# ChampiB/CBO_with_OOP

Measured on AMD Instinct MI355X. Metric: candidate-intervention acquisitions/sec (16k grid, d=3), higher is better.
Workload: dtype f64

## Files before the change

cbo_with_oop_amd/csrc/cbo_api.hip:

```cpp
#include <algorithm>
#include <atomic>
#include <cmath>
#include <cstdio>
#include <cstdlib>
#include <chrono>
#include <cstring>
#include <mutex>
#include <string>
#include <map>
#include <utility>
#include <vector>

#include "cbo_internal.h"
#include "schedule_tuner.h"

using namespace cbo;

static thread_local std::string g_err;
static std::atomic<uint64_t> g_fit_stamp{0};

static int fail(int code, const std::string &msg)
{
    g_err = msg;
    return code;
}
namespace cbo {
int set_error(int code, const std::string &msg) { return fail(code, msg); }
}

static std::mutex g_live_mutex;
static std::vector<cbo_ctx *> g_live;
static void shutdown_all_at_exit()
{
    for (;;) {
        cbo_ctx *c = nullptr;
        {
            std::lock_guard<std::mutex> lock(g_live_mutex);
            if (g_live.empty()) break;
            c = g_live.back();
        }
        cbo_shutdown(c);
    }
}

#define HIP_TRY(expr)                                                                                   \
    do {                                                                                                \
        hipError_t e_ = (expr);                                                                         \
        if (e_ != hipSuccess)                                                                           \
            return fail(CBO_ERR_HIP, std::string(#expr) + ": " + hipGetErrorString(e_));                \
    } while (0)

constexpr size_t kStageBytes = 64 << 10;

enum Phase { PH_KXX = 0, PH_CHOL, PH_ALPHA, PH_KSTAR, PH_TRSM, PH_ACQ, PH_CONVERT, PH_COUNT };

struct EventPair {
    hipEvent_t a, b;
    int phase;
};

template <class T, bool Pinned = false>
struct GrowBuf {
    T *p = nullptr;
    size_t cap = 0;
    GrowBuf() = default;
    GrowBuf(const GrowBuf &) = delete;
    GrowBuf &operator=(const GrowBuf &) = delete;
    ~GrowBuf() { release(); }
    operator T *() const { return p; }
    void release() { if (p) Pinned ? hipHostFree(p) : hipFree(p); p = nullptr; cap = 0; }
};
template <class T>
using PinnedBuf = GrowBuf<T, true>;

struct cbo_ctx {
    int device = 0;
    hipStream_t stream = nullptr;
    hipStream_t side_stream = nullptr;
    hipStream_t sweep_stream = nullptr;
    hipStream_t bulk_stream = nullptr;
    std::vector<hipEvent_t> chol_events;
    std::vector<hipEvent_t> pipe_events;
    hipEvent_t ev_join = nullptr, ev_join2 = nullptr, ev_fork = nullptr;
    hipEvent_t region_a = nullptr, region_b = nullptr;
    double pipe_tail_frac = -1.0;
    int pipe_group = 0;
    int pipe_lead = -1;
    CholOptions chol;
    int vec_solve_form = 2;
    int n_cu = 256;
    int n_cu_pipe = 256;
    ScheduleTable schedule;
    int64_t fused_fallbacks = 0;
    bool sweep_cache = true;
    bool small_sets = true;
    int sweep_mode = -1;
    int overlap_mode = -1;
    bool profiling = false;
    std::vector<EventPair> pending;
    EventPair pipe_cur{};
    std::vector<hipEvent_t> pool;
    cbo_timers timers{};
    GrowBuf<double> V;
    GrowBuf<double> W;
    GrowBuf<double> gpart;
    GrowBuf<double> mupart;
    PinnedBuf<cbo_small_set> sets_host;
    PinnedBuf<cbo_small_result> small_out;
    GrowBuf<double> small_scratch;
    GrowBuf<double> small_part_val; GrowBuf<int64_t> small_part_idx;
    GrowBuf<int> small_info;
    int small_seq = 0;
    int polled_launches = 0;
    PinnedBuf<cbo_small_lml_result> lml_out;
    PinnedBuf<cbo_small_lml_result> lml_batch_out;
    PinnedBuf<cbo_small_loo_result> loo_out;
    int loo_route = 0;
    PinnedBuf<double> hyper_host;
    PinnedBuf<HyperSet> hyper_sets_host;
    GrowBuf<double> hyper_sum;
    PinnedBuf<cbo_small_aux> aux_host;
    PinnedBuf<double> mes_host;
    GrowBuf<double> gumbel_mean, gumbel_var, gumbel_out;
    GrowBuf<int64_t> gumbel_status;
    PinnedBuf<GumbelSet> gumbel_sets_host;
    int hyper_schedule = 0;
    GrowBuf<double> q, mu, mean, var, acq;
    double *part_val = nullptr; int64_t *part_idx = nullptr;
    double *best_val = nullptr; int64_t *best_idx = nullptr;
    double *h_best_val = nullptr; int64_t *h_best_idx = nullptr;
    int *h_info = nullptr;
    cbo_cands *scratch_k = nullptr;
    GrowBuf<double> grads;
    GrowBuf<double> export_buf;
    GrowBuf<double> cov;
    GrowBuf<double> samp_A, samp_invDt;
    GrowBuf<int> samp_info;
    GrowBuf<double> samp_Z, samp_out;
    GrowBuf<double> ivr_part;
    GrowBuf<double> con_terms;
    GrowBuf<double> plugin_y;
    GrowBuf<double> batch_W, batch_q, batch_col, batch_part;
    GrowBuf<double> append_part;
    GrowBuf<BatchState> batch_state;
    PinnedBuf<double> batch_h_vals; PinnedBuf<int64_t> batch_h_idxs;
    double *stage = nullptr; hipEvent_t stage_done = nullptr; bool stage_pending = false;
    size_t max_ws_bytes = (size_t)32 << 30;
    char name[128] = {0};
};

struct cbo_gp {
    cbo_ctx *ctx = nullptr;
    int64_t n = 0, n_pad = 0, lda = 0;
    int d = 0;
    PointSet X;
    double *raw = nullptr;
    double *y = nullptr, *ls_dev = nullptr;
    std::vector<double> ls;
    std::vector<double> h_pv;
    KernelHyper h{};
    double noise_var = 0.0;
    double *A = nullptr;
    double *invDt = nullptr;
    double *alpha = nullptr;
    double *z = nullptr;
    int *info = nullptr;
    bool fitted = false;
    uint64_t fit_stamp = 0;
    bool alpha_ready = false;
    int tries = 0;
    double jitter = 0.0;
    uint64_t parent_stamp = 0;
    double append_d = 0.0, append_zn = 0.0;
    double *lvec = nullptr;
    cbo_cands *probe = nullptr;
    int k_last = 1;
// ... 103 lines not shown
        float ms = 0.f;
        hipEventElapsedTime(&ms, p.a, p.b);
        switch (p.phase) {
            case PH_KXX: c->timers.ms_kxx += ms; break;
            case PH_CHOL: c->timers.ms_chol += ms; break;
            case PH_ALPHA: c->timers.ms_alpha += ms; break;
            case PH_KSTAR: c->timers.ms_kstar += ms; break;
            case PH_TRSM: c->timers.ms_trsm += ms; break;
            case PH_ACQ: c->timers.ms_acq += ms; break;
            case PH_CONVERT: c->timers.ms_f32_convert += ms; break;
        }
        c->pool.push_back(p.a);
        c->pool.push_back(p.b);
    }
    c->pending.clear();
}

static void destroy_ctx(cbo_ctx *c);

extern "C" int cbo_abi_version(void) { return CBO_HIP_ABI_VERSION; }
extern "C" const char *cbo_last_error(void) { return g_err.c_str(); }

extern "C" int cbo_device_count(int *count_out)
{
    if (!count_out) return fail(CBO_ERR_INVALID, "count_out is NULL");
    int n = 0;
    hipError_t e = hipGetDeviceCount(&n);
    if (e != hipSuccess) { (void)hipGetLastError(); n = 0; }
    *count_out = n;
    return CBO_OK;
}

extern "C" int cbo_init(int device_id, cbo_ctx **out)
{
    if (!out) return fail(CBO_ERR_INVALID, "out is NULL");
    int n = 0;
    if (hipGetDeviceCount(&n) != hipSuccess || n <= 0) {
        (void)hipGetLastError();
        return fail(CBO_ERR_NO_DEVICE, "no HIP device visible: libcbo_hip has no CPU fallback");
    }
    if (device_id < 0 || device_id >= n) return fail(CBO_ERR_INVALID, "device_id out of range");
    HIP_TRY(hipSetDevice(device_id));
    hipDeviceProp_t prop;
    HIP_TRY(hipGetDeviceProperties(&prop, device_id));
    if (std::strncmp(prop.gcnArchName, "gfx950", 6) != 0)
        return fail(CBO_ERR_NO_DEVICE, std::string("device is ") + prop.gcnArchName +
                                           ", this library carries gfx950 code objects only");
    cbo_ctx *c = new cbo_ctx();
    c->device = device_id;
    std::snprintf(c->name, sizeof(c->name), "%s (%s, %d CUs)", prop.name, prop.gcnArchName, prop.multiProcessorCount);
    int prio_low = 0, prio_high = 0;
    hipError_t e = hipDeviceGetStreamPriorityRange(&prio_low, &prio_high);
    if (e == hipSuccess) e = hipStreamCreateWithPriority(&c->stream, hipStreamNonBlocking, prio_high);
    if (e == hipSuccess)
        e = hipStreamCreateWithPriority(&c->side_stream, hipStreamNonBlocking, (prio_low + prio_high) / 2);
    if (e == hipSuccess) {
        constexpr int reserve = 4;
        const int n_cu = prop.multiProcessorCount;
        std::vector<uint32_t> mask((size_t)(n_cu + 31) / 32, 0u);
        for (int b = 0; b < n_cu; ++b)
            if (b / 8 >= reserve) mask[(size_t)b / 32] |= 1u << (b % 32);
        bool masked = false;
        c->n_cu_pipe = n_cu;
        if (reserve * 8 < n_cu) {
            masked = hipExtStreamCreateWithCUMask(&c->sweep_stream, (uint32_t)mask.size(), mask.data()) == hipSuccess &&
                     hipExtStreamCreateWithCUMask(&c->bulk_stream, (uint32_t)mask.size(), mask.data()) == hipSuccess;
            if (masked) c->n_cu_pipe = n_cu - reserve * 8;
            if (!masked) {
                (void)hipGetLastError();
                if (c->sweep_stream) { hipStreamDestroy(c->sweep_stream); c->sweep_stream = nullptr; }
                if (c->bulk_stream) { hipStreamDestroy(c->bulk_stream); c->bulk_stream = nullptr; }
            }
        }
        if (!masked) {
            e = hipStreamCreateWithPriority(&c->sweep_stream, hipStreamNonBlocking, (prio_low + prio_high) / 2);
            if (e == hipSuccess) e = hipStreamCreateWithPriority(&c->bulk_stream, hipStreamNonBlocking, prio_low);
        }
    }
    if (e == hipSuccess) e = hipEventCreateWithFlags(&c->ev_join, hipEventDisableTiming | hipEventDisableSystemFence);
    if (e == hipSuccess) e = hipEventCreateWithFlags(&c->ev_join2, hipEventDisableTiming | hipEventDisableSystemFence);
    if (e == hipSuccess) e = hipEventCreateWithFlags(&c->ev_fork, hipEventDisableTiming | hipEventDisableSystemFence);
    if (e == hipSuccess) e = hipMalloc(&c->part_val, 2048 * sizeof(double));
    if (e == hipSuccess) e = hipMalloc(&c->part_idx, 2048 * sizeof(int64_t));
    if (e == hipSuccess) e = hipMalloc(&c->best_val, sizeof(double));
    if (e == hipSuccess) e = hipMalloc(&c->best_idx, sizeof(int64_t));
    if (e == hipSuccess) e = hipHostMalloc(&c->h_best_val, sizeof(double));
    if (e == hipSuccess) e = hipHostMalloc(&c->h_best_idx, sizeof(int64_t));
    if (e == hipSuccess) e = hipHostMalloc(&c->h_info, sizeof(int));
    if (e == hipSuccess) e = hipHostMalloc(&c->stage, kStageBytes);
    if (e == hipSuccess) e = hipEventCreateWithFlags(&c->stage_done, hipEventDisableTiming);
    if (e != hipSuccess) {
        destroy_ctx(c);
        return fail(CBO_ERR_HIP, std::string("cbo_init: ") + hipGetErrorString(e));
    }
    const char *ws = std::getenv("CBO_HIP_WORKSPACE_MB");
    if (ws) c->max_ws_bytes = (size_t)std::atoll(ws) << 20;
    c->n_cu = prop.multiProcessorCount;
    const char *sm = std::getenv("CBO_HIP_SWEEP");
    if (sm) c->sweep_mode = std::atoi(sm);
    const char *lr = std::getenv("CBO_HIP_LOO_ROUTE");
    if (lr) c->loo_route = std::atoi(lr);
    const char *hs = std::getenv("CBO_HIP_HYPER_SCHEDULE");
    if (hs) c->hyper_schedule = std::atoi(hs);
    const char *sc = std::getenv("CBO_HIP_SWEEP_CACHE");
    if (sc && std::atoi(sc) == 0) c->sweep_cache = false;
    const char *ss = std::getenv("CBO_HIP_SMALL_SETS");
    if (ss && std::atoi(ss) == 0) c->small_sets = false;
    const char *om = std::getenv("CBO_HIP_OVERLAP");
    if (om) c->overlap_mode = std::atoi(om);
    const char *tf = std::getenv("CBO_HIP_PIPE_TAIL");
    if (tf) c->pipe_tail_frac = std::atof(tf);
    const char *pg = std::getenv("CBO_HIP_PIPE_GROUP");
    if (pg) c->pipe_group = std::min(std::max(std::atoi(pg), 0), 4);
    const char *pl = std::getenv("CBO_HIP_PIPE_LEAD");
    if (pl) c->pipe_lead = std::atoi(pl);
    const char *pf = std::getenv("CBO_HIP_PANEL_FORM");
    if (pf && (std::atoi(pf) == 2 || std::atoi(pf) == 5)) c->chol.panel_form = std::atoi(pf);
    const char *sl = std::getenv("CBO_HIP_FUSED_SPIN_LIMIT");
    if (sl) c->chol.spin_limit = std::atoi(sl);
    const char *bg = std::getenv("CBO_HIP_BULK_GROUP");
    if (bg) c->chol.bulk_group = std::atoi(bg);
    const char *g4 = std::getenv("CBO_HIP_BULK_GROUP4_ROWS");
    if (g4) c->chol.group4_rows = std::atoi(g4);
    const char *vf = std::getenv("CBO_HIP_VEC_SOLVE_FORM");
    if (vf) c->vec_solve_form = std::atoi(vf);
    {
        static std::once_flag once;
        std::call_once(once, [] { std::atexit(shutdown_all_at_exit); });
        std::lock_guard<std::mutex> lock(g_live_mutex);
        g_live.push_back(c);
    }
    *out = c;
    return CBO_OK;
}

namespace cbo {
hipStream_t ctx_stream(cbo_ctx *c) { return c->stream; }
int ctx_device(cbo_ctx *c) { return c->device; }
}

extern "C" void cbo_shutdown(cbo_ctx *c)
{
    if (!c) return;
    {
        std::lock_guard<std::mutex> lock(g_live_mutex);
        auto it = std::find(g_live.begin(), g_live.end(), c);
        if (it == g_live.end()) return;
        g_live.erase(it);
    }
    destroy_ctx(c);
}

static void destroy_ctx(cbo_ctx *c)
{
    hipSetDevice(c->device);
    if (c->scratch_k) { cbo_cands_destroy(c->scratch_k); c->scratch_k = nullptr; }
    if (c->stream) hipStreamSynchronize(c->stream);
    for (auto &p : c->pending) { hipEventDestroy(p.a); hipEventDestroy(p.b); }
    for (auto e : c->pool) hipEventDestroy(e);
    hipFree(c->part_val); hipFree(c->part_idx); hipFree(c->best_val); hipFree(c->best_idx);
    hipHostFree(c->h_best_val); hipHostFree(c->h_best_idx); hipHostFree(c->h_info); hipHostFree(c->stage);
    if (c->stage_done) hipEventDestroy(c->stage_done);
    for (auto e : c->chol_events) hipEventDestroy(e);
    for (auto e : c->pipe_events) hipEventDestroy(e);
    if (c->region_a) hipEventDestroy(c->region_a);
    if (c->region_b) hipEventDestroy(c->region_b);
    if (c->ev_join) hipEventDestroy(c->ev_join);
    if (c->ev_join2) hipEventDestroy(c->ev_join2);
    if (c->ev_fork) hipEventDestroy(c->ev_fork);
    if (c->sweep_stream) hipStreamDestroy(c->sweep_stream);
    if (c->bulk_stream) hipStreamDestroy(c->bulk_stream);
    if (c->side_stream) hipStreamDestroy(c->side_stream);
    if (c->stream) hipStreamDestroy(c->stream);
    delete c;
}

extern "C" int cbo_synchronize(cbo_ctx *c)
{
    if (!c) return fail(CBO_ERR_INVALID, "ctx is NULL");
    HIP_TRY(hipSetDevice(c->device));
    HIP_TRY(hipDeviceSynchronize());
    return CBO_OK;
}

extern "C" int cbo_set_profiling(cbo_ctx *c, int enabled)
{
    if (!c) return fail(CBO_ERR_INVALID, "ctx is NULL");
    c->profiling = enabled != 0;
    return CBO_OK;
}

extern "C" int cbo_reset_timers(cbo_ctx *c)
{
    if (!c) return fail(CBO_ERR_INVALID, "ctx is NULL");
    resolve_events(c);
    c->timers = cbo_timers{};
    return CBO_OK;
}

extern "C" int cbo_get_timers(cbo_ctx *c, cbo_timers *out)
{
    if (!c || !out) return fail(CBO_ERR_INVALID, "NULL argument");
    resolve_events(c);
    *out = c->timers;
    return CBO_OK;
}

extern "C" int cbo_region_begin(cbo_ctx *c)
{
    if (!c) return fail(CBO_ERR_INVALID, "ctx is NULL");
    HIP_TRY(hipSetDevice(c->device));
    if (!c->region_a) {
        HIP_TRY(hipEventCreate(&c->region_a));
        HIP_TRY(hipEventCreate(&c->region_b));
    }
    HIP_TRY(hipEventRecord(c->region_a, c->stream));
    return CBO_OK;
}

extern "C" int cbo_region_end(cbo_ctx *c, double *ms_out)
{
    if (!c || !ms_out) return fail(CBO_ERR_INVALID, "NULL argument");
    if (!c->region_a) return fail(CBO_ERR_INVALID, "cbo_region_end without cbo_region_begin");
    HIP_TRY(hipSetDevice(c->device));
    HIP_TRY(hipEventRecord(c->region_b, c->stream));
    HIP_TRY(hipEventSynchronize(c->region_b));
    float ms = 0.f;
    HIP_TRY(hipEventElapsedTime(&ms, c->region_a, c->region_b));
    *ms_out = ms;
    return CBO_OK;
}

extern "C" int cbo_device_name(cbo_ctx *c, char *buf, int buflen)
{
    if (!c || !buf || buflen <= 0) return fail(CBO_ERR_INVALID, "NULL argument");
    std::snprintf(buf, (size_t)buflen, "%s", c->name);
    return CBO_OK;
}

static void free_gp_data(cbo_gp *g)
{
    hipFree(g->X.xs); hipFree(g->X.sq); hipFree(g->X.sv); hipFree(g->X.pm); hipFree(g->X.pv);
// ... 72 lines not shown
        return CBO_OK;
    }
    HIP_TRY(hipMemcpyAsync(g->raw, X, sizeof(double) * n * g->d, hipMemcpyHostToDevice, c->stream));
    HIP_TRY(hipMemcpyAsync(g->y, y, sizeof(double) * n, hipMemcpyHostToDevice, c->stream));
    g->h_pv.clear();
    if (pv) {
        HIP_TRY(hipMemcpyAsync(g->X.pm, pm, sizeof(double) * n, hipMemcpyHostToDevice, c->stream));
        HIP_TRY(hipMemcpyAsync(g->X.pv, pv, sizeof(double) * n, hipMemcpyHostToDevice, c->stream));
        g->h_pv.assign(pv, pv + n);
    }
    launch_prep_points(c->stream, g->raw, n, g->d, g->h.ard ? g->ls_dev : nullptr, pv ? g->X.pv : nullptr, g->X.xs,
                       n_pad, g->X.sq, g->X.sv);
    HIP_TRY(hipGetLastError());
    HIP_TRY(hipStreamSynchronize(c->stream));
    return CBO_OK;
}

extern "C" int cbo_gp_create(cbo_ctx *c, int dtype, int64_t n, int d, const double *X, const double *y,
                             const double *pm, const double *pv, double variance, const double *lengthscale,
                             int ard, double noise_var, int zero_diag, cbo_gp **out)
{
    if (!c || !out || !lengthscale) return fail(CBO_ERR_INVALID, "NULL argument");
    if (dtype != CBO_DTYPE_F64 && dtype != CBO_DTYPE_F32) return fail(CBO_ERR_INVALID, "dtype must be CBO_DTYPE_F64 or CBO_DTYPE_F32");
    if (d < 1 || d > CBO_MAX_DIM) return fail(CBO_ERR_INVALID, "d must be in [1, CBO_MAX_DIM]");
    HIP_TRY(hipSetDevice(c->device));
    cbo_gp *g = new cbo_gp();
    g->ctx = c;
    g->d = d;
    g->dtype = dtype;
    g->noise_var = noise_var;
    g->h.variance = variance;
    g->h.ard = ard ? 1 : 0;
    g->h.zero_diag = zero_diag ? 1 : 0;
    g->h.lengthscale = ard ? 1.0 : lengthscale[0];
    g->ls.assign(lengthscale, lengthscale + (ard ? d : 1));
    if (hipMalloc(&g->info, sizeof(int) * (1 + kCholFlagSlots)) != hipSuccess) { delete g; return fail(CBO_ERR_HIP, "hipMalloc info"); }
    if (ard) {
        if (hipMalloc(&g->ls_dev, sizeof(double) * d) != hipSuccess ||
            hipMemcpy(g->ls_dev, lengthscale, sizeof(double) * d, hipMemcpyHostToDevice) != hipSuccess) {
            cbo_gp_destroy(g);
            return fail(CBO_ERR_HIP, "hipMalloc/hipMemcpy lengthscales");
        }
    }
    const int rc = upload_gp_data(g, n, X, y, pm, pv);
    if (rc != CBO_OK) { cbo_gp_destroy(g); return rc; }
    *out = g;
    return CBO_OK;
}

extern "C" void cbo_gp_destroy(cbo_gp *g)
{
    if (g && g->probe) { cbo_cands_destroy(g->probe); g->probe = nullptr; }
    if (!g) return;
    for (cbo_cands *&p : g->blk_probe)
        if (p) { cbo_cands_destroy(p); p = nullptr; }
    hipSetDevice(g->ctx->device);
    hipStreamSynchronize(g->ctx->stream);
    hipFree(g->blk_mem);
    free_gp_data(g);
    hipFree(g->info);
    hipFree(g->ls_dev); hipFree(g->inv_ls_dev);
    delete g;
}

extern "C" int64_t cbo_gp_n(const cbo_gp *g) { return g ? g->n : -1; }
extern "C" int cbo_gp_dtype(const cbo_gp *g) { return g ? g->dtype : -1; }

extern "C" int cbo_gp_jitter(const cbo_gp *g, int *tries_out, double *jitter_out)
{
    if (!g) return fail(CBO_ERR_INVALID, "gp is NULL");
    if (!g->fitted) return fail(CBO_ERR_NOT_FITTED, "gp is not fitted");
    if (tries_out) *tries_out = g->tries;
    if (jitter_out) *jitter_out = g->jitter;
    return CBO_OK;
}

static CholOptions chol_options(const cbo_ctx *c, bool separate)
{
    CholOptions o = c->chol;
    if (separate) o.panel_form = 2;
    return o;
}

static void enqueue_factor(cbo_gp *g, double jitter, bool separate)
{
    cbo_ctx *c = g->ctx;
    {
        PhaseScope ps(c, PH_KXX);
        launch_kxx(c->stream, g->X, g->h, g->noise_var + kGpyDiagJitter, jitter, g->A, g->lda, g->n_pad);
        launch_rhs(c->stream, g->y, g->X.pm, g->n, g->A, g->lda, g->n_pad, g->info, cholesky_info_ints(g->n_pad));
    }
    {
        PhaseScope ps(c, PH_CHOL);
        launch_cholesky(c->stream, c->side_stream, c->chol_events, g->A, g->lda, g->n_pad, g->invDt, g->info,
                        chol_options(c, separate), nullptr, true);
    }
}

static bool jitter_step(double base, int *tries, double *jitter)
{
    *jitter = *tries == 0 ? base : *jitter * 10.0;
    ++*tries;
    return *tries <= 5 && std::isfinite(*jitter);
}

static int next_jitter(cbo_gp *g, int *tries, double *jitter)
{
    double base = 0.0;
    if (*tries == 0) {
        long double sum = 0.0L;
        bool nonpos = false;
        for (int64_t i = 0; i < g->n; ++i) {
            const double dv = g->h.variance + (g->h_pv.empty() ? 0.0 : g->h_pv[i]) + (g->noise_var + kGpyDiagJitter);
            if (!(dv > 0.0)) nonpos = true;
            sum += (long double)dv;
        }
        if (nonpos) return fail(CBO_ERR_NONPOS_DIAG, "not pd: non-positive diagonal elements");
        base = (double)(sum / (long double)g->n) * 1e-6;
    }
    if (!jitter_step(base, tries, jitter)) return fail(CBO_ERR_NOT_PD, "not positive definite, even with jitter.");
    return CBO_OK;
}

template <class Enqueue>
static int attempt_factor(cbo_ctx *c, const int *info, Enqueue enqueue, bool *pd)
{
    for (bool separate = false;;) {
        enqueue(separate);
        HIP_TRY(hipGetLastError());
        HIP_TRY(hipMemcpyAsync(c->h_info, info, sizeof(int), hipMemcpyDeviceToHost, c->stream));
        HIP_TRY(hipStreamSynchronize(c->stream));
        if (*c->h_info == kCholFusedTimeout) {
            if (separate)
                return fail(CBO_ERR_HIP, "a fused diagonal + panel launch gave up waiting, and so did the separate-launch repeat");
            separate = true;
            ++c->fused_fallbacks;
            continue;
        }
        *pd = *c->h_info == 0;
        return CBO_OK;
    }
}

static void mark_fitted(cbo_gp *g, int tries, double jitter)
{
    g->fitted = true;
    g->fit_stamp = ++g_fit_stamp;
    g->parent_stamp = 0;
    g->alpha_ready = false;
    g->tries = tries;
    g->jitter = jitter;
    if (g->ctx->profiling) g->ctx->timers.n_fit += 1;
}

static int adopt_factor(cbo_gp *g, int tries, double jitter)
{
    cbo_ctx *c = g->ctx;
    HIP_TRY(hipMemcpy2DAsync(g->z, sizeof(double), g->A + g->n_pad, sizeof(double) * g->lda, sizeof(double),
                             (size_t)g->n_pad, hipMemcpyDeviceToDevice, c->stream));
    HIP_TRY(hipGetLastError());
    mark_fitted(g, tries, jitter);
    return CBO_OK;
}

extern "C" int cbo_gp_fit(cbo_gp *g, int *tries_out, double *jitter_out)
{
    if (!g) return fail(CBO_ERR_INVALID, "gp is NULL");
    if (g->n <= 0 || g->n_pad <= 0) return fail(CBO_ERR_INVALID, "gp holds no data (a previous upload failed)");
    cbo_ctx *c = g->ctx;
    HIP_TRY(hipSetDevice(c->device));
    g->fitted = false;
    double jitter = 0.0;
    int tries = 0;
    for (;;) {
        bool pd = false;
        int rc = attempt_factor(c, g->info, [&](bool separate) { enqueue_factor(g, jitter, separate); }, &pd);
        if (rc != CBO_OK) return rc;
        if (pd) break;
// ... 350 lines not shown
static bool prefer_right_looking(const cbo_ctx *c, int64_t n_pad, int64_t cols)
{
    if (c->sweep_mode == 0) return false;
    if (c->sweep_mode == 1) return true;
    if (n_pad < 1024) return false;
    const int64_t strips = cols / kStrip;
    const int64_t rounds = (strips + c->n_cu - 1) / c->n_cu;
    return rounds * c->n_cu * 5 >= strips * 6;
}


static int enqueue_right_looking(cbo_gp *g, double *V, int64_t ldv, int64_t cols, double *q, double *mu,
                                 bool lower_tri = false)
{
    cbo_ctx *c = g->ctx;
    SweepPipe pipe = make_pipe(g, V, ldv, cols, q, mu);
    pipe.lower_tri = lower_tri;
    HIP_TRY(hipMemsetAsync(q, 0, sizeof(double) * cols, c->stream));
    HIP_TRY(hipMemsetAsync(mu, 0, sizeof(double) * cols, c->stream));
    int p = 0;
    for (int r0 = 0; r0 < (int)g->n_pad; r0 += 256, ++p)
        sweep_pipe_pair(pipe, c->stream, g->A, g->lda, g->invDt, g->n_pad, p, r0,
                        (r0 + 256 <= (int)g->n_pad) ? 256 : 128);
    HIP_TRY(hipEventRecord(c->ev_join, c->sweep_stream));
    HIP_TRY(hipStreamWaitEvent(c->stream, c->ev_join, 0));
    HIP_TRY(hipEventRecord(c->ev_join2, c->bulk_stream));
    HIP_TRY(hipStreamWaitEvent(c->stream, c->ev_join2, 0));
    return CBO_OK;
}

static int own_solution_buffer(cbo_gp *g, cbo_cands *k, double **V, int64_t *ldv)
{
    cbo_ctx *c = g->ctx;
    if (!k->V || k->v_rows_cap != g->n_pad || k->v_ld != k->m_pad + kLdExtra) {
        HIP_TRY(hipStreamSynchronize(c->stream));
        hipFree(k->V); hipFree(k->partial);
        k->V = nullptr; k->partial = nullptr; k->v_stamp = 0;
        k->v_ld = k->m_pad + kLdExtra;
        HIP_TRY(hipMalloc(&k->V, sizeof(double) * (size_t)g->n_pad * (size_t)k->v_ld));
        HIP_TRY(hipMalloc(&k->partial, sizeof(double) * 64 * (size_t)k->m_pad));
        k->v_rows_cap = g->n_pad;
    }
    *V = k->V;
    *ldv = k->v_ld;
    return CBO_OK;
}

static int enqueue_posterior_f32(cbo_gp *g, cbo_cands *k)
{
    cbo_ctx *c = g->ctx;
    int64_t chunk = 0, ldv = 0;
    int rc = ensure_workspaces(c, g->n32, k->m_pad, &chunk, &ldv, sizeof(float));
    if (rc != CBO_OK) return rc;
    rc = ensure_alpha(g);
    if (rc != CBO_OK) return rc;
    rc = grow(c, c->mupart, (size_t)(g->n32 / 64) * (size_t)chunk);
    if (rc != CBO_OK) return rc;
    if (g->f32_stamp != g->fit_stamp) {
        PhaseScope ps(c, PH_CONVERT);
        launch_factor_to_f32(c->stream, g->A, g->lda, g->n_pad, g->invDt, g->Uf, g->ldu32, g->invF, g->n32);
        g->f32_stamp = g->fit_stamp;
    }
    float *Vf = reinterpret_cast<float *>(c->V.p);
    k->v_stamp = 0;
    for (int64_t c0 = 0; c0 < k->m_pad; c0 += chunk) {
        const int64_t cols = (k->m_pad - c0 < chunk) ? (k->m_pad - c0) : chunk;
        {
            PhaseScope ps(c, PH_KSTAR);
            launch_kstar_f32(c->stream, g->X, k->P, c0, cols, g->h, Vf, ldv, g->n32, g->alpha, c->mupart, c->mu + c0);
        }
        {
            PhaseScope ps(c, PH_TRSM);
            launch_trsm_strips_f32(c->stream, g->Uf, g->ldu32, g->invF, Vf, ldv, g->n32, cols, c->q + c0);
        }
        if (c->profiling) {
            c->timers.n_trsm_launches += 1;
            c->timers.trsm_flops += (double)g->n32 * (double)g->n32 * (double)cols;
        }
    }
    HIP_TRY(hipGetLastError());
    return CBO_OK;
}

static int solve_columns(cbo_gp *g, const cbo_cands *k, int64_t c_begin, int64_t cols, double *V, int64_t ldv, double *q,
                         double *mu)
{
    cbo_ctx *c = g->ctx;
    {
        PhaseScope ps(c, PH_KSTAR);
        launch_kstar(c->stream, g->X, k->P, c_begin, cols, g->h, V, ldv, g->n_pad);
    }
    if (prefer_right_looking(c, g->n_pad, cols)) return enqueue_right_looking(g, V, ldv, cols, q, mu);
    {
        PhaseScope ps(c, PH_TRSM);
        launch_trsm_strips(c->stream, g->A, g->lda, g->invDt, V, ldv, g->n_pad, cols, g->z, q, mu);
    }
    if (c->profiling) {
        c->timers.n_trsm_launches += 1;
        c->timers.trsm_flops += (double)g->n_pad * (double)g->n_pad * (double)cols;
    }
    return CBO_OK;
}

static int enqueue_posterior(cbo_gp *g, cbo_cands *k, bool want_f64_solution = false)
{
    cbo_ctx *c = g->ctx;
    int rc = prepare_cands(g, k);
    if (rc != CBO_OK) return rc;
    if (g->dtype == CBO_DTYPE_F32 && !want_f64_solution) return enqueue_posterior_f32(g, k);
    int64_t chunk = 0, ldv = 0;
    rc = ensure_workspaces(c, g->n_pad, k->m_pad, &chunk, &ldv);
    if (rc != CBO_OK) return rc;
    double *Vws = c->V;
    k->v_stamp = 0;
    if (k->keep_v && chunk >= k->m_pad) {
        rc = own_solution_buffer(g, k, &Vws, &ldv);
        if (rc != CBO_OK) return rc;
    }
    for (int64_t c0 = 0; c0 < k->m_pad; c0 += chunk) {
        const int64_t cols = (k->m_pad - c0 < chunk) ? (k->m_pad - c0) : chunk;
        rc = solve_columns(g, k, c0, cols, Vws, ldv, c->q + c0, c->mu + c0);
        if (rc != CBO_OK) return rc;
    }
    HIP_TRY(hipGetLastError());
    if (Vws != c->V) { k->v_stamp = g->fit_stamp; k->v_rows = g->n; }
    return CBO_OK;
}

static int check_sweep_args(const cbo_gp *g, const cbo_cands *k, int task)
{
    if (!g || !k) return fail(CBO_ERR_INVALID, "NULL argument");
    if (g->ctx != k->ctx) return fail(CBO_ERR_INVALID, "gp and candidates live on different contexts");
    if (g->d != k->d) return fail(CBO_ERR_INVALID, "gp and candidates have different dimensions");
    if ((g->X.sv != nullptr) && !k->has_prior)
        return fail(CBO_ERR_INVALID, "causal gp needs candidate prior mean/variance");
    if (task != CBO_TASK_MIN && task != CBO_TASK_MAX) return fail(CBO_ERR_INVALID, "task must be 0 (min) or 1 (max)");
    return CBO_OK;
}

static int copy_posterior_out(cbo_ctx *c, const cbo_cands *k, double *acq_out, double *mean_out, double *var_out)
{
    if (acq_out) HIP_TRY(hipMemcpyAsync(acq_out, c->acq, sizeof(double) * k->m, hipMemcpyDeviceToHost, c->stream));
    if (mean_out) HIP_TRY(hipMemcpyAsync(mean_out, c->mean, sizeof(double) * k->m, hipMemcpyDeviceToHost, c->stream));
    if (var_out) HIP_TRY(hipMemcpyAsync(var_out, c->var, sizeof(double) * k->m, hipMemcpyDeviceToHost, c->stream));
    return CBO_OK;
}

static int enqueue_finish(cbo_gp *g, cbo_cands *k, double y_best, int task, double ei_jitter, double cost, double *acq_out,
                          double *mean_out, double *var_out, const double *q_src, const double *mu_src,
                          bool with_status = false, bool copy_out = true, const MesParams *mes = nullptr, int kind = 0,
                          const double *y_best_dev = nullptr)
{
    cbo_ctx *c = g->ctx;
    const bool causal = g->X.sv != nullptr;
    AcqParams p;
    p.variance = g->h.variance; p.noise_var = g->noise_var; p.y_best = y_best; p.ei_jitter = ei_jitter; p.cost = cost;
    p.task = task; p.include_noise = 1; p.want_ei = 1;
    p.y_best_dev = y_best_dev;
    const int nb = acq_blocks_for(k->m);
    {
        PhaseScope ps(c, PH_ACQ);
        if (mes)
            launch_mes_acq(c->stream, q_src, mu_src, causal ? k->pm : nullptr, causal ? k->pv : nullptr, k->m, *mes,
                           mean_out ? c->mean : nullptr, var_out ? c->var : nullptr, acq_out ? c->acq : nullptr,
                           c->part_val, c->part_idx, k->index_offset, nb);
        else if (kind == CBO_ACQ_LCB || kind == CBO_ACQ_PI || kind == CBO_ACQ_VAR)
            launch_pointwise_acq(c->stream, kind, q_src, mu_src, causal ? k->pm : nullptr, causal ? k->pv : nullptr, k->m, p,
                                 mean_out ? c->mean : nullptr, var_out ? c->var : nullptr, acq_out ? c->acq : nullptr,
                                 c->part_val, c->part_idx, k->index_offset, nb);
        else
            launch_acq(c->stream, q_src, mu_src, causal ? k->pm : nullptr, causal ? k->pv : nullptr, k->m, p,
                       mean_out ? c->mean : nullptr, var_out ? c->var : nullptr, acq_out ? c->acq : nullptr, c->part_val,
                       c->part_idx, k->index_offset, nb);
        launch_argmax_final(c->stream, c->part_val, c->part_idx, nb, c->h_best_val, c->h_best_idx,
                            with_status ? g->info : nullptr, with_status ? c->h_info : nullptr);
    }
    HIP_TRY(hipGetLastError());
    if (copy_out) return copy_posterior_out(c, k, acq_out, mean_out, var_out);
    return CBO_OK;
}

static void complete_finish(cbo_ctx *c, double *best_val, int64_t *best_idx)
{
    if (best_val) *best_val = *c->h_best_val;
    if (best_idx) *best_idx = *c->h_best_idx;
    if (c->profiling) c->timers.n_sweep += 1;
}

static int settle_vectors(cbo_gp *g, cbo_cands *k, bool own, const double **q_src, const double **mu_src)
{
    cbo_ctx *c = g->ctx;
    const bool cached = k->fit_stamp != 0 && k->fit_stamp == g->fit_stamp;
    if (!cached && (c->sweep_cache || own)) {
        const int rc = cands_cache_vectors(k);
        if (rc != CBO_OK) return rc;
        HIP_TRY(hipMemcpyAsync(k->q, c->q, sizeof(double) * k->m_pad, hipMemcpyDeviceToDevice, c->stream));
        HIP_TRY(hipMemcpyAsync(k->mu, c->mu, sizeof(double) * k->m_pad, hipMemcpyDeviceToDevice, c->stream));
        if (c->sweep_cache) k->fit_stamp = g->fit_stamp;
    }
    *q_src = (cached || own) ? k->q : c->q;
    *mu_src = (cached || own) ? k->mu : c->mu;
    return CBO_OK;
}

static int finish_sweep(cbo_gp *g, cbo_cands *k, double y_best, int task, double ei_jitter, double cost,
                        double *acq_out, double *mean_out, double *var_out, double *best_val, int64_t *best_idx,
                        const MesParams *mes = nullptr, int kind = 0, const double *y_best_dev = nullptr)
{
    cbo_ctx *c = g->ctx;
    const double *q_src = nullptr, *mu_src = nullptr;
    int rc = settle_vectors(g, k, false, &q_src, &mu_src);
    if (rc != CBO_OK) return rc;
    rc = enqueue_finish(g, k, y_best, task, ei_jitter, cost, acq_out, mean_out, var_out, q_src, mu_src, false, true, mes,
                        kind, y_best_dev);
    if (rc != CBO_OK) return rc;
    HIP_TRY(hipStreamSynchronize(c->stream));
    complete_finish(c, best_val, best_idx);
    return CBO_OK;
}

static int extend_solution_by_one_row(cbo_gp *g, cbo_cands *k)
{
    cbo_ctx *c = g->ctx;
    int rc = prepare_cands(g, k);
    if (rc != CBO_OK) return rc;
    int64_t chunk = 0, ldv = 0;
    rc = ensure_workspaces(c, g->n_pad, k->m_pad, &chunk, &ldv);
    if (rc != CBO_OK) return rc;
    if (chunk < k->m_pad) return CBO_OK;
    const int64_t row = g->n - 1;
    PointSet one = g->probe->P;
    one.n = 1;
    launch_kstar(c->stream, one, k->P, 0, k->m_pad, g->h, c->V, ldv, 64);
    launch_append_row(c->stream, k->V, k->v_ld, row, g->lvec, k->m_pad, c->V, g->append_d, g->append_zn, k->partial,
                      k->q, k->mu);
    HIP_TRY(hipGetLastError());
    k->v_rows = g->n;
    k->v_stamp = g->fit_stamp;
    k->fit_stamp = g->fit_stamp;
    return CBO_OK;
}

extern "C" int cbo_cands_keep_solution(cbo_cands *k, int on)
{
    if (!k) return fail(CBO_ERR_INVALID, "cands is NULL");
    k->keep_v = on != 0;
    if (!k->keep_v) {
        hipSetDevice(k->ctx->device);
        hipStreamSynchronize(k->ctx->stream);
        hipFree(k->V); hipFree(k->partial);
        k->V = nullptr; k->partial = nullptr; k->v_stamp = 0; k->v_rows_cap = 0;
    }
    return CBO_OK;
}

extern "C" int cbo_gp_append(cbo_gp *g, const double *x_new, double y_new, double prior_mean_new, double prior_var_new,
                             int *appended_out)
{
    if (!g || !x_new || !appended_out) return fail(CBO_ERR_INVALID, "NULL argument");
    *appended_out = 0;
    if (!g->fitted) return fail(CBO_ERR_NOT_FITTED, "gp is not fitted");
    if (g->tries != 0 || g->n >= g->n_pad) return CBO_OK;
    if (g->dtype != CBO_DTYPE_F64) return CBO_OK;
    cbo_ctx *c = g->ctx;
    HIP_TRY(hipSetDevice(c->device));
    const bool causal = g->X.sv != nullptr;
    if (g->probe) {
        cbo_cands *p = g->probe;
        HIP_TRY(hipMemcpyAsync(p->raw, x_new, sizeof(double) * g->d, hipMemcpyHostToDevice, c->stream));
        if (causal) {
            HIP_TRY(hipMemcpyAsync(p->pm, &prior_mean_new, sizeof(double), hipMemcpyHostToDevice, c->stream));
            HIP_TRY(hipMemcpyAsync(p->pv, &prior_var_new, sizeof(double), hipMemcpyHostToDevice, c->stream));
        }
        HIP_TRY(hipStreamSynchronize(c->stream));
        p->prepared_for = nullptr;
        p->fit_stamp = 0;
    } else {
        int rc = cbo_cands_create(c, 1, g->d, x_new, causal ? &prior_mean_new : nullptr, causal ? &prior_var_new : nullptr,
                                  0, &g->probe);
        if (rc != CBO_OK) return rc;
    }
    int rc = prepare_cands(g, g->probe);
    if (rc != CBO_OK) return rc;
    int64_t chunk = 0, ldv = 0;
    rc = ensure_workspaces(c, g->n_pad, g->probe->m_pad, &chunk, &ldv);
    if (rc != CBO_OK) return rc;
    launch_kstar(c->stream, g->X, g->probe->P, 0, g->probe->m_pad, g->h, c->V, ldv, g->n_pad);
    launch_gather_column(c->stream, c->V, ldv, g->n_pad, g->alpha + g->n_pad);
    const bool chained = launch_forward_chain(c->stream, g->A, g->lda, g->n_pad, g->invDt, g->alpha + g->n_pad, g->lvec,
                                              g->info, c->chol.spin_limit, c->vec_solve_form);
    if (!chained) launch_forward_vec(c->stream, g->A, g->lda, g->n_pad, g->invDt, g->alpha + g->n_pad, g->lvec);
    HIP_TRY(hipGetLastError());
    launch_dot2(c->stream, g->lvec, g->z, g->n, c->part_val);
    HIP_TRY(hipGetLastError());
    double hd[2];
    HIP_TRY(hipMemcpyAsync(hd, c->part_val, sizeof(hd), hipMemcpyDeviceToHost, c->stream));
    if (chained) HIP_TRY(hipMemcpyAsync(c->h_info, g->info, sizeof(int), hipMemcpyDeviceToHost, c->stream));
// ... 94 lines not shown
    if (causal) {
        HIP_TRY(hipMemcpyAsync(p->pm, prior_mean_new, sizeof(double) * k, hipMemcpyHostToDevice, c->stream));
        HIP_TRY(hipMemcpyAsync(p->pv, prior_var_new, sizeof(double) * k, hipMemcpyHostToDevice, c->stream));
    }
    HIP_TRY(hipMemcpyAsync(g->blk_y[side], y_new, sizeof(double) * k, hipMemcpyHostToDevice, c->stream));
    rc = prepare_cands(g, p);
    if (rc != CBO_OK) return rc;
    int64_t chunk = 0, ldv = 0;
    rc = ensure_workspaces(c, g->n_pad, p->m_pad, &chunk, &ldv);
    if (rc != CBO_OK) return rc;
    const int kp = (int)round_up(k, 16);
    const int64_t ldk = kAppendLd + kLdExtra;
    launch_kstar(c->stream, g->X, p->P, 0, p->m_pad, g->h, c->V, ldv, g->n_pad);
    PointSet pb = p->P;
    pb.n = k;
    launch_kstar(c->stream, pb, p->P, 0, p->m_pad, g->h, g->blk_Kbb[side], ldk, 64);
    launch_append_forward(c->stream, g->A, g->lda, g->n_pad, g->invDt, c->V, ldv, kp, g->blk_B[side]);
    AppendSchurArgs sa{};
    sa.part = g->blk_part; sa.k = k;
    sa.Kbb = g->blk_Kbb[side]; sa.ldk = ldk;
    sa.pv = causal ? p->pv : nullptr; sa.pm = causal ? p->pm : nullptr;
    sa.y_new = g->blk_y[side];
    sa.variance = g->h.variance; sa.sigma = g->noise_var + kGpyDiagJitter;
    sa.L22 = g->blk_L22[side]; sa.zb = g->blk_zb[side]; sa.status = g->blk_status;
    launch_append_schur(c->stream, g->blk_B[side], g->n, g->z, sa);
    HIP_TRY(hipGetLastError());
    HIP_TRY(hipMemcpyAsync(c->h_info, g->blk_status, sizeof(int), hipMemcpyDeviceToHost, c->stream));
    HIP_TRY(hipStreamSynchronize(c->stream));
    if (*c->h_info != 0) return CBO_OK;
    HIP_TRY(hipMemcpyAsync(g->raw + g->n * g->d, p->raw, sizeof(double) * k * g->d, hipMemcpyDeviceToDevice, c->stream));
    AppendCommitArgs ca{};
    ca.A = g->A; ca.lda = g->lda; ca.n = g->n; ca.n_pad = g->n_pad; ca.k = k;
    ca.B = g->blk_B[side]; ca.L22 = g->blk_L22[side]; ca.zb = g->blk_zb[side]; ca.y_new = g->blk_y[side];
    ca.z = g->z; ca.y = g->y;
    ca.dims = g->X.d; ca.xs = g->X.xs; ca.ldx = g->X.ld; ca.sq = g->X.sq; ca.sv = g->X.sv; ca.pm = g->X.pm; ca.pv = g->X.pv;
    ca.pxs = p->P.xs; ca.ldp = p->P.ld; ca.psq = p->P.sq; ca.psv = p->P.sv; ca.pm_new = p->pm; ca.pv_new = p->pv;
    launch_append_block_commit(c->stream, ca, g->invDt);
    HIP_TRY(hipGetLastError());
    HIP_TRY(hipStreamSynchronize(c->stream));
    if (causal) g->h_pv.insert(g->h_pv.end(), prior_var_new, prior_var_new + k);
    g->n += k;
    g->X.n = g->n;
    g->k_last = k;
    g->blk_side = side;
    g->parent_stamp = g->fit_stamp;
    g->fit_stamp = ++g_fit_stamp;
    g->alpha_ready = false;
    *appended_out = 1;
    return CBO_OK;
}

static int extend_solution_by_block(cbo_gp *g, cbo_cands *k)
{
    cbo_ctx *c = g->ctx;
    int rc = prepare_cands(g, k);
    if (rc != CBO_OK) return rc;
    int64_t chunk = 0, ldv = 0;
    rc = ensure_workspaces(c, g->n_pad, k->m_pad, &chunk, &ldv);
    if (rc != CBO_OK) return rc;
    if (chunk < k->m_pad) return CBO_OK;
    const int kb = g->k_last, kp = (int)round_up(kb, 16), side = g->blk_side;
    const int64_t n0 = g->n - kb;
    int slices = 1, rps = 64;
    append_rows_plan(n0, k->m_pad, &slices, &rps);
    rc = grow(c, c->append_part, (size_t)slices * (size_t)kp * (size_t)k->m_pad);
    if (rc != CBO_OK) return rc;
    PointSet pb = g->blk_probe[side]->P;
    pb.n = kb;
    launch_kstar(c->stream, pb, k->P, 0, k->m_pad, g->h, c->V, ldv, 64);
    AppendRowsArgs ra{};
    ra.k = kb; ra.m_pad = k->m_pad;
    ra.Kb = c->V; ra.ldk = ldv;
    ra.L22 = g->blk_L22[side]; ra.zb = g->blk_zb[side];
    ra.Vnew = k->V + n0 * k->v_ld; ra.ldv = k->v_ld;
    ra.q = k->q; ra.mu = k->mu;
    launch_append_rows(c->stream, k->V, k->v_ld, g->blk_B[side], n0, kp, c->append_part, ra);
    HIP_TRY(hipGetLastError());
    k->v_rows = g->n;
    k->v_stamp = g->fit_stamp;
    k->fit_stamp = g->fit_stamp;
    return CBO_OK;
}

static int enqueue_vectors(cbo_gp *g, cbo_cands *k, bool *substituted = nullptr)
{
    int rc = CBO_OK;
    cbo_ctx *c = g->ctx;
    if (k->keep_v && k->V && k->v_stamp != 0 && k->v_stamp == g->parent_stamp && k->v_rows == g->n - g->k_last &&
        k->v_rows_cap == g->n_pad && k->fit_stamp == k->v_stamp && k->q) {
        rc = g->k_last == 1 ? extend_solution_by_one_row(g, k) : extend_solution_by_block(g, k);
        if (rc != CBO_OK) return rc;
    }
    if (!(c->sweep_cache && k->fit_stamp != 0 && k->fit_stamp == g->fit_stamp)) {
        k->fit_stamp = 0;
        if (substituted) *substituted = true;
        return enqueue_posterior(g, k);
    }
    return grow_vectors(c, k->m_pad);
}

static int sweep_impl(cbo_gp *g, cbo_cands *k, double y_best, int task, double ei_jitter, double cost, double *acq_out,
                      double *mean_out, double *var_out, double *best_val, int64_t *best_idx, const MesParams *mes,
                      int kind = 0, const double *y_best_dev = nullptr)
{
    HIP_TRY(hipSetDevice(g->ctx->device));
    const int rc = enqueue_vectors(g, k);
    if (rc != CBO_OK) return rc;
    return finish_sweep(g, k, y_best, task, ei_jitter, cost, acq_out, mean_out, var_out, best_val, best_idx, mes, kind,
                        y_best_dev);
}

extern "C" int cbo_acq_sweep(cbo_gp *g, cbo_cands *k, double y_best, int task, double ei_jitter, double cost,
                             double *acq_out, double *mean_out, double *var_out, double *best_val, int64_t *best_idx)
{
    int rc = check_sweep_args(g, k, task);
    if (rc != CBO_OK) return rc;
    if (!g->fitted) return fail(CBO_ERR_NOT_FITTED, "gp is not fitted");
    return sweep_impl(g, k, y_best, task, ei_jitter, cost, acq_out, mean_out, var_out, best_val, best_idx, nullptr);
}

extern "C" int cbo_acq_sweep_batch(cbo_gp *g, cbo_cands *k, double y_best, int task, double ei_jitter, double cost,
                                   int batch_size, int update_incumbent, double *best_vals, int64_t *best_idxs,
                                   double *acq_out, double *mean_out, double *var_out)
{
    int rc = check_sweep_args(g, k, task);
    if (rc != CBO_OK) return rc;
    if (batch_size < 1 || batch_size > CBO_MAX_BATCH)
        return fail(CBO_ERR_INVALID, "batch_size must be in 1.." + std::to_string(CBO_MAX_BATCH));
    if (batch_size > k->m) return fail(CBO_ERR_INVALID, "batch_size exceeds the number of candidates");
    if (!best_vals || !best_idxs) return fail(CBO_ERR_INVALID, "NULL argument");
    if (!(cost > 0.0)) return fail(CBO_ERR_INVALID, "cost must be positive");
    if (update_incumbent != 0 && update_incumbent != 1) return fail(CBO_ERR_INVALID, "update_incumbent must be 0 or 1");
    if (!g->fitted) return fail(CBO_ERR_NOT_FITTED, "gp is not fitted");
    cbo_ctx *c = g->ctx;
    HIP_TRY(hipSetDevice(c->device));
    const bool f32 = g->dtype == CBO_DTYPE_F32;
    if (batch_size == 1 && !f32)
        return sweep_impl(g, k, y_best, task, ei_jitter, cost, acq_out, mean_out, var_out, best_vals, best_idxs, nullptr);
    int64_t chunk = 0, ld_ws = 0;
    rc = ensure_workspaces(c, g->n_pad, k->m_pad, &chunk, &ld_ws);
    if (rc != CBO_OK) return rc;
    if (batch_size > 1 && chunk < k->m_pad)
        return fail(CBO_ERR_UNSUPPORTED, "cbo_acq_sweep_batch needs L^-1 K* of all " + std::to_string(k->m_pad) +
                                             " padded candidates resident at once; the workspace holds " +
                                             std::to_string(chunk) + " columns: raise CBO_HIP_WORKSPACE_MB");
    const double *q_src = nullptr, *mu_src = nullptr;
    bool substituted = false;
    if (f32) {
        rc = enqueue_posterior(g, k, true);
        substituted = true;
        q_src = c->q; mu_src = c->mu;
    } else {
        rc = enqueue_vectors(g, k, &substituted);
        if (rc == CBO_OK) rc = settle_vectors(g, k, false, &q_src, &mu_src);
    }
    if (rc != CBO_OK) return rc;
    auto kept = [&] {
        return k->keep_v && k->V && k->v_stamp != 0 && k->v_stamp == g->fit_stamp && k->v_rows == g->n &&
               k->v_rows_cap == g->n_pad;
    };
    const double *V = nullptr;
    int64_t ldv = 0;
    if (batch_size > 1) {
        if (!kept() && !substituted) {
            rc = enqueue_posterior(g, k);
            if (rc != CBO_OK) return rc;
        }
        if (kept()) { V = k->V; ldv = k->v_ld; }
        else { V = c->V; ldv = ld_ws; }
    }
    const int64_t m_pad = k->m_pad;
    rc = grow(c, c->batch_state, 1);
    if (rc == CBO_OK) rc = grow(c, c->batch_h_vals, CBO_MAX_BATCH);
    if (rc == CBO_OK) rc = grow(c, c->batch_h_idxs, CBO_MAX_BATCH);
    if (rc == CBO_OK && batch_size > 1) rc = grow(c, c->batch_W, (size_t)(batch_size - 1) * (size_t)m_pad);
    if (rc == CBO_OK && batch_size > 1) rc = grow(c, c->batch_q, (size_t)m_pad);
    if (rc == CBO_OK && batch_size > 1) rc = grow(c, c->batch_col, (size_t)g->n_pad);
    if (rc == CBO_OK && batch_size > 1) rc = grow(c, c->batch_part, (size_t)batch_slices(g->n) * (size_t)m_pad);
    if (rc != CBO_OK) return rc;
    const bool causal = g->X.sv != nullptr;
    const double *pm = causal ? k->pm : nullptr, *pv = causal ? k->pv : nullptr;
    AcqParams p;
    p.variance = g->h.variance; p.noise_var = g->noise_var; p.y_best = y_best; p.ei_jitter = ei_jitter; p.cost = cost;
    p.task = task; p.include_noise = 1; p.want_ei = 1;
    const int nb = acq_blocks_for(k->m);
    {
        PhaseScope ps(c, PH_ACQ);
        launch_batch_state_init(c->stream, c->batch_state, y_best);
        const double *q_cur = q_src;
        for (int t = 0; t < batch_size; ++t) {
            const bool last = t == batch_size - 1;
            if (t == 1)
// ... 139 lines not shown
    complete_finish(c, best_val, best_idx);
    return CBO_OK;
}

extern "C" int cbo_gp_fit_sweep(cbo_gp *g, cbo_cands *k, double y_best, int task, double ei_jitter, double cost,
                                double *acq_out, double *mean_out, double *var_out, double *best_val,
                                int64_t *best_idx, int *tries_out, double *jitter_out)
{
    int rc = check_sweep_args(g, k, task);
    if (rc != CBO_OK) return rc;
    if (g->n <= 0 || g->n_pad <= 0) return fail(CBO_ERR_INVALID, "gp holds no data (a previous upload failed)");
    cbo_ctx *c = g->ctx;
    HIP_TRY(hipSetDevice(c->device));
    if (g->dtype == CBO_DTYPE_F32) {
        rc = cbo_gp_fit(g, tries_out, jitter_out);
        if (rc != CBO_OK) return rc;
        return cbo_acq_sweep(g, k, y_best, task, ei_jitter, cost, acq_out, mean_out, var_out, best_val, best_idx);
    }
    rc = prepare_cands(g, k);
    if (rc != CBO_OK) return rc;
    int64_t chunk = 0, ldv = 0;
    rc = ensure_workspaces(c, g->n_pad, k->m_pad, &chunk, &ldv);
    if (rc != CBO_OK) return rc;
    if (chunk < k->m_pad) {
        rc = cbo_gp_fit(g, tries_out, jitter_out);
        if (rc != CBO_OK) return rc;
        return cbo_acq_sweep(g, k, y_best, task, ei_jitter, cost, acq_out, mean_out, var_out, best_val, best_idx);
    }
    using clk = std::chrono::steady_clock;
    const clk::time_point t_call = clk::now();
    auto us_since = [](clk::time_point a) { return std::chrono::duration<double, std::micro>(clk::now() - a).count(); };
    const int nb = (int)(g->n_pad / 128);
    const int all_pairs = (nb + 1) / 2;
    const bool forced = c->overlap_mode == 0 || c->overlap_mode == 1 || c->pipe_tail_frac >= 0.0 || c->pipe_group != 0 ||
                        all_pairs < 2;
    ScheduleEntry *entry = nullptr;
    ScheduleChoice choice;
    if (forced) {
        choice.group = c->pipe_group >= 2 ? c->pipe_group : (c->pipe_group == 0 && k->m_pad / kStrip >= c->n_cu_pipe) ? 2 : 0;
        if (c->overlap_mode == 0 || (all_pairs < 2 && c->overlap_mode != 1)) choice.pairs = kSequence;
        else if (c->pipe_tail_frac >= 0.0) {
            int tail_blocks = (int)(c->pipe_tail_frac * nb + 0.5);
            tail_blocks += (nb - tail_blocks) & 1;
            choice.pairs = (nb - (tail_blocks > nb ? nb : tail_blocks)) / 2;
        } else choice.pairs = all_pairs >= 4 ? all_pairs / 4 : 1;
    } else {
        entry = &schedule_entry(c->schedule, c->n_cu_pipe, g->n_pad, k->m_pad / kStrip, k->m_pad);
        choice = schedule_choose(*entry, !c->profiling, c->n_cu, c->n_cu_pipe);
        entry->ran_pairs = choice.pairs;
        entry->ran_group = choice.pairs > 0 ? choice.group : 0;
    }
    if (choice.pairs == kSequence) {
        int tries = 0;
        double jitter = 0.0;
        const clk::time_point t_fit = clk::now();
        rc = cbo_gp_fit(g, &tries, &jitter);
        if (tries_out) *tries_out = tries;
        if (jitter_out) *jitter_out = jitter;
        if (rc != CBO_OK) return rc;
        const double fact_us = us_since(t_fit);
        const clk::time_point t_sweep = clk::now();
        rc = cbo_acq_sweep(g, k, y_best, task, ei_jitter, cost, acq_out, mean_out, var_out, best_val, best_idx);
        if (rc == CBO_OK && entry)
            schedule_report(c->n_cu, c->n_cu_pipe, *entry, choice, tries, us_since(t_call) * 1e-3, fact_us, us_since(t_sweep));
        return rc;
    }
    g->fitted = false;
    double *Vws = c->V;
    k->v_stamp = 0;
    if (k->keep_v) {
        rc = own_solution_buffer(g, k, &Vws, &ldv);
        if (rc != CBO_OK) return rc;
    }
    double *qbuf = c->q, *mubuf = c->mu;
    if (c->sweep_cache) {
        rc = cands_cache_vectors(k);
        if (rc != CBO_OK) return rc;
        qbuf = k->q;
        mubuf = k->mu;
        k->fit_stamp = 0;
    }
    const bool speculate = qbuf == k->q;
    SweepPipe pipe = make_pipe(g, Vws, ldv, k->m_pad, qbuf, mubuf);
    pipe.group = choice.group;
    int pairs = choice.pairs;
    pipe.lead = 0;
    if (pipe.group >= 2 && pairs >= 1 && pairs * 256 < (int)g->n_pad)
        pipe.lead = forced ? (c->pipe_lead > 0 ? c->pipe_lead : 0) : (c->pipe_lead >= 0 ? c->pipe_lead : pairs % pipe.group);
    pipe.tail_begin = pairs * 256;
    if (pipe.tail_begin > (int)g->n_pad) pipe.tail_begin = (int)g->n_pad;
    double jitter = 0.0;
    int tries = 0;
    bool separate = false;
    for (;;) {
        HIP_TRY(hipEventRecord(c->ev_fork, c->stream));
        HIP_TRY(hipStreamWaitEvent(c->sweep_stream, c->ev_fork, 0));
        {
            PhaseScope ps(c, PH_KXX);
            launch_kxx(c->stream, g->X, g->h, g->noise_var + kGpyDiagJitter, jitter, g->A, g->lda, g->n_pad);
            launch_rhs(c->stream, g->y, g->X.pm, g->n, g->A, g->lda, g->n_pad, g->info, cholesky_info_ints(g->n_pad));
        }
        {
            PhaseScope ps(c, PH_KSTAR, c->sweep_stream);
            launch_kstar(c->sweep_stream, g->X, k->P, 0, k->m_pad, g->h, Vws, ldv, g->n_pad);
        }
        launch_zero_pair(c->sweep_stream, qbuf, mubuf, k->m_pad);
        {
            PhaseScope ps(c, PH_CHOL);
            launch_cholesky(c->stream, c->side_stream, c->chol_events, g->A, g->lda, g->n_pad, g->invDt, g->info,
                            chol_options(c, separate), &pipe, true);
        }
        HIP_TRY(hipEventRecord(c->ev_join, c->sweep_stream));
        HIP_TRY(hipStreamWaitEvent(c->stream, c->ev_join, 0));
        HIP_TRY(hipEventRecord(c->ev_join2, c->bulk_stream));
        HIP_TRY(hipStreamWaitEvent(c->stream, c->ev_join2, 0));
        HIP_TRY(hipGetLastError());
        if (speculate) {
            rc = enqueue_finish(g, k, y_best, task, ei_jitter, cost, acq_out, mean_out, var_out, qbuf, mubuf, true, false);
            if (rc != CBO_OK) return rc;
        } else {
            HIP_TRY(hipMemcpyAsync(c->h_info, g->info, sizeof(int), hipMemcpyDeviceToHost, c->stream));
        }
        HIP_TRY(hipStreamSynchronize(c->stream));
        if (*c->h_info == 0) break;
        if (*c->h_info == kCholFusedTimeout) {
            if (separate)
                return fail(CBO_ERR_HIP, "a fused diagonal + panel launch gave up waiting, and so did the separate-launch repeat");
            separate = true;
            ++c->fused_fallbacks;
            continue;
        }
        rc = next_jitter(g, &tries, &jitter);
        if (rc != CBO_OK) return rc;
    }
    mark_fitted(g, tries, jitter);
    if (tries_out) *tries_out = tries;
    if (jitter_out) *jitter_out = jitter;
    if (Vws != c->V) { k->v_stamp = g->fit_stamp; k->v_rows = g->n; }
    if (qbuf == k->q) k->fit_stamp = g->fit_stamp;
    if (speculate) {
        if (acq_out || mean_out || var_out) {
            rc = copy_posterior_out(c, k, acq_out, mean_out, var_out);
            if (rc != CBO_OK) return rc;
            HIP_TRY(hipStreamSynchronize(c->stream));
        }
        complete_finish(c, best_val, best_idx);
        if (entry) schedule_report(c->n_cu, c->n_cu_pipe, *entry, choice, separate ? -1 : tries, us_since(t_call) * 1e-3, 0.0, 0.0);
        return CBO_OK;
    }
    rc = finish_sweep(g, k, y_best, task, ei_jitter, cost, acq_out, mean_out, var_out, best_val, best_idx);
    if (rc == CBO_OK && entry)
        schedule_report(c->n_cu, c->n_cu_pipe, *entry, choice, separate ? -1 : tries, us_since(t_call) * 1e-3, 0.0, 0.0);
    return rc;
}

constexpr double kPollBudgetUs = 2000.0;
constexpr int kPolledLaunchesPerSync = 256;
template <class Pred>
static bool poll_until(Pred done, double budget_us)
{
    using clk = std::chrono::steady_clock;
    const clk::time_point t0 = clk::now();
    for (;;) {
        for (int spin = 0; spin < 256; ++spin)
            if (done()) return true;
        if (std::chrono::duration<double, std::micro>(clk::now() - t0).count() > budget_us) return done();
    }
}

template <class Rec, class Launch>
static int polled_launch(cbo_ctx *c, const char *name, const Rec *out, int n, const char *missing, Launch launch)
{
    if (++c->small_seq == 0) c->small_seq = 1;
    const int seq = c->small_seq;
    static const bool trace_slow = std::getenv("CBO_HIP_TRACE_SLOW") != nullptr;
    static const double trace_over_us = trace_slow && std::atof(std::getenv("CBO_HIP_TRACE_SLOW")) > 1.0
                                            ? std::atof(std::getenv("CBO_HIP_TRACE_SLOW")) : 1000.0;
    using clk = std::chrono::steady_clock;
    const clk::time_point t_begin = trace_slow ? clk::now() : clk::time_point();
    const int rc = launch(seq);
    if (rc != CBO_OK) return rc;
    const clk::time_point t_launched = trace_slow ? clk::now() : clk::time_point();
    const bool all = poll_until([&] {
        for (int j = 0; j < n; ++j)
            if (*reinterpret_cast<const volatile int *>(&out[j].seq) != seq) return false;
        return true;
    }, kPollBudgetUs);
    const clk::time_point t_polled = trace_slow ? clk::now() : clk::time_point();
    const bool reap = ++c->polled_launches >= kPolledLaunchesPerSync;
    if (reap) c->polled_launches = 0;
    if (!all || c->profiling || reap) HIP_TRY(hipStreamSynchronize(c->stream));
    if (trace_slow) {
        const clk::time_point t_end = clk::now();
        auto us = [](clk::time_point a, clk::time_point b) { return std::chrono::duration<double, std::micro>(b - a).count(); };
        if (us(t_begin, t_end) > trace_over_us)
            std::fprintf(stderr, "[cbo] slow %s call #%d: launch %.1f us, poll %.1f us (%s), synchronise %.1f us (%s)\n",
                         name, seq, us(t_begin, t_launched), us(t_launched, t_polled), all ? "records arrived" : "gave up",
                         us(t_polled, t_end), !all ? "after the poll gave up" : reap ? "periodic reap" : "none");
    }
    for (int j = 0; j < n; ++j)
// ... 1721 lines not shown
```

cbo_with_oop_amd/csrc/cbo_internal.h:

```cpp
#pragma once

#include <hip/hip_runtime.h>
#include <cstddef>
#include <cstdint>
#include <string>
#include <vector>

#include "cbo_hip.h"

namespace cbo {

typedef double d4 __attribute__((ext_vector_type(4)));
typedef double d2 __attribute__((ext_vector_type(2)));

#if defined(__HIP_DEVICE_COMPILE__) || defined(__HIPCC__)
typedef __attribute__((address_space(3))) void *lds_ptr_t;
__device__ __forceinline__ void glds16(const double *gsrc, unsigned lds_dst)
{
    unsigned keep;
    asm volatile("s_mov_b32 %0, m0\n\ts_mov_b32 m0, %2\n\ts_nop 0\n\tglobal_load_lds_dwordx4 %1, off\n\ts_mov_b32 m0, %0"
                 : "=&s"(keep)
                 : "v"(gsrc), "s"(lds_dst)
                 : "memory");
}
__device__ __forceinline__ unsigned lds_byte_address(const void *p)
{
    return (unsigned)(unsigned long)(lds_ptr_t)p;
}
#endif

constexpr int kPadN = 128;
constexpr int kStrip = 64;
constexpr int kRhsCols = 64;
constexpr int kLdExtra = 16;

inline int64_t round_up(int64_t v, int64_t m) { return (v + m - 1) / m * m; }

int set_error(int code, const std::string &msg);
hipStream_t ctx_stream(cbo_ctx *c);
int ctx_device(cbo_ctx *c);
int gp_factor_view(cbo_gp *g, double **A, int64_t *lda, int64_t *n_pad, double **invDt, cbo_ctx **ctx);
bool gp_is_fitted_at(const cbo_gp *g, int level);
int gp_adopt_received_factor(cbo_gp *g, int level);

constexpr double kGpyDiagJitter = 1e-8;
constexpr double kGpyVarClip = 1e-15;

struct PointSet {
    double *xs = nullptr;
    double *sq = nullptr;
    double *sv = nullptr;
    double *pm = nullptr;
    double *pv = nullptr;
    int64_t n = 0, ld = 0;
    int d = 0;
};

struct KernelHyper {
    double variance;
    double lengthscale;
    int ard;
    int zero_diag;
};

void launch_prep_points(hipStream_t s, const double *raw_aos, int64_t n, int d, const double *ls_dev ,
                        const double *pv_raw , double *xs, int64_t ld, double *sq, double *sv);

void launch_prep_points_staged(hipStream_t s, const double *stage, int64_t n, int d, const double *ls_dev, bool has_prior,
                               double *raw, double *y, double *pm, double *pv, double *xs, int64_t ld, double *sq,
                               double *sv);

void launch_kxx(hipStream_t s, const PointSet &X, const KernelHyper &h, double diag_add, double jitter,
                double *A, int64_t lda, int64_t n_pad);
void launch_zero_pair(hipStream_t s, double *a, double *b, int64_t n);
void launch_rhs(hipStream_t s, const double *y, const double *pm, int64_t n, double *A, int64_t lda, int64_t n_pad,
                int *zero = nullptr, int zero_count = 0);
void launch_kstar(hipStream_t s, const PointSet &X, const PointSet &C, int64_t c_begin, int64_t m_pad,
                  const KernelHyper &h, double *V, int64_t ldv, int64_t n_pad);

struct CovArgs {
    const double *V; int64_t ldv;
    int64_t a_off, b_off, v_cols;
    int n_k;
    const double *xs1, *sq1, *sv1, *xs2, *sq2, *sv2; int64_t ldx;
    int64_t m1, m2;
    double *C; int64_t ldc;
    double variance, inv_l2, noise;
    int zero_diag, tiles;
};
void launch_cov_tiles(hipStream_t s, int d, bool sym, CovArgs a);
struct SampArgs {
    const double *U; int64_t ldu;
    const double *Z; int64_t ldz;
    const double *mean;
    int64_t m, s;
    double *F; int64_t ldf;
    int tiles_i, tiles_j;
};
void launch_samples_tiles(hipStream_t st, SampArgs a);
void launch_normals_transpose(hipStream_t st, const double *normals, int64_t m, int64_t s, double *Z, int64_t m_pad,
                              int64_t ldz);
void launch_factor_padding(hipStream_t st, double *A, int64_t lda, int64_t m, int64_t m_pad);
constexpr int kJointTile = 128;
struct IvrArgs {
    const double *Vc, *Vi; int64_t ldv, c_cols, i_cols;
    int n_k;
    const double *xs1, *sq1, *sv1, *xs2, *sq2, *sv2; int64_t ldx;
    int64_t m, p;
    double *part; int64_t ldp; int64_t tile0;
    double variance, inv_l2;
};
void launch_ivr_tiles(hipStream_t s, int d, IvrArgs a);
void launch_ivr_finish(hipStream_t s, const double *part, int64_t ldp, int tiles, const double *var, int64_t m, double p,
                       double cost, double *ivr, double *part_val, int64_t *part_idx, int n_blocks);
int ivr_finish_blocks_for(int64_t m);
constexpr int kPadN32 = 256;
void launch_factor_to_f32(hipStream_t s, const double *A, int64_t lda, int64_t n_pad, const double *invDt, float *Uf,
                          int64_t ldu, float *invF, int64_t n32);
void launch_kstar_f32(hipStream_t s, const PointSet &X, const PointSet &C, int64_t c_begin, int64_t m_pad,
                      const KernelHyper &h, float *V, int64_t ldv, int64_t n32, const double *alpha, double *mu_part,
                      double *mu);
void launch_trsm_strips_f32(hipStream_t s, const float *U, int64_t ldu, const float *invDt, float *V, int64_t ldv,
                            int64_t n32, int64_t m_pad, double *q);
int run_mfma_f32_selftest(hipStream_t s, double *max_err);

struct SweepPipe {
    hipStream_t stream;
    hipStream_t bulk;
    double *V;
    int64_t ldv, m_pad;
    double *zvec;
    double *q, *mu;
    bool lower_tri;
    int group;
    int lead = 0;
    int tail_begin;
    std::vector<hipEvent_t> *events;
    void (*mark)(void *user, hipStream_t st, int begin, double flops);
    void *user;
};
constexpr int kCholFlagSlots = 1024;
constexpr int kCholFusedTimeout = -2147483647 - 1;
constexpr int kFusedSpinLimit = 1 << 22;
struct CholOptions {
    int panel_form = 4;
    int spin_limit = kFusedSpinLimit;
    int bulk_group = 4;
    int group4_rows = 10240;
};
void launch_cholesky(hipStream_t s, hipStream_t side, std::vector<hipEvent_t> &events, double *A, int64_t lda,
                     int64_t n_pad, double *invDt, int *info_dev, const CholOptions &opt, const SweepPipe *pipe = nullptr,
                     bool info_zeroed = false);
inline int cholesky_info_ints(int64_t n_pad)
{
    const int np = (int)(n_pad / 128);
    return 2 * np <= kCholFlagSlots ? 1 + 2 * np : 1;
}
void sweep_pipe_pair(const SweepPipe &pipe, hipStream_t chain, const double *A, int64_t lda, const double *invDt,
                     int64_t n_pad, int p, int r0, int klen);
void sweep_pipe_tail(const SweepPipe &pipe, hipStream_t chain, const double *A, int64_t lda, const double *invDt,
                     int64_t n_pad, int pairs_done);
void launch_backsolve(hipStream_t s, const double *A, int64_t lda, int64_t n_pad, const double *invDt, double *alpha);
void launch_forward_vec(hipStream_t s, const double *A, int64_t lda, int64_t n_pad, const double *invDt, double *w,
                        double *out);
void launch_gather_column(hipStream_t s, const double *V, int64_t ldv, int64_t n_pad, double *dst);
bool launch_backsolve_chain(hipStream_t s, const double *A, int64_t lda, int64_t n_pad, const double *invDt,
                            const double *src, int64_t src_stride, double *work, double *out, int *info, int spin_limit,
                            int form);
bool launch_forward_chain(hipStream_t s, const double *A, int64_t lda, int64_t n_pad, const double *invDt, const double *w,
                          double *out, int *info, int spin_limit, int form);
void launch_backsolve_vec(hipStream_t s, const double *A, int64_t lda, int64_t n_pad, const double *invDt,
                          const double *src, int64_t src_stride, double *work, double *out);
void launch_pred_gradients(hipStream_t s, const PointSet &X, int64_t n_pad, const PointSet &C, int64_t c_begin,
                           int64_t cols, int64_t m, const KernelHyper &h, const double *inv_ls_dev, const double *alpha,
                           const double *W, int64_t ldw, double *dmean, double *dvar);
void launch_reversed_factor(hipStream_t s, const double *A, int64_t lda, int64_t n_pad, const double *invDt, double *T,
                            int64_t ldt, double *invT);
void launch_reverse_rows(hipStream_t s, const double *V, int64_t ldv, int64_t n_pad, int64_t cols, double *W, int64_t ldw);
void launch_dot2(hipStream_t s, const double *a, const double *b, int64_t n, double *out2);
void launch_sum(hipStream_t s, const double *a, int64_t n, double *out);
void launch_expand_interventions(hipStream_t s, const double *observed, int64_t n_obs, int d, const double *values, int n_iv,
                                 const int *iv_index, int64_t m, double *raw);

void launch_trsm_strips(hipStream_t s, const double *U, int64_t ldu, const double *invDt, double *V, int64_t ldv,
                        int64_t n, int64_t m_pad, const double *z, double *q, double *mu, bool accumulate = false,
                        bool half_lds = false);
void launch_gemm_update(hipStream_t s, const double *U, int64_t ldu, const double *V, int64_t ldv, double *C,
                        int64_t ldc, int k0, int klen, int i0_begin, int i0_end, int64_t m_pad, bool upper_only,
                        const int *skip_if = nullptr);

struct cbo_small_set {
    const double *xs, *sq, *sv, *pm, *y;
    const double *cxs, *csq, *csv, *cpm, *cpv;
    int64_t ld, cld, m, index_offset;
    int n, d, zero_diag, task;
    double variance, lengthscale, noise_var, diag_add, y_best, ei_jitter, cost;
    int ard, pad_;
    const double *stage, *stage_ls;
    double *raw, *pv;
};
struct cbo_small_result {
    double best_val;
    int64_t best_idx;
    int info;
    int seq;
};
size_t small_sets_scratch_doubles(int n_sets, int blocks_per_set);
constexpr int kSmallLmlTerms = 1 + CBO_MAX_DIM + 4;
struct cbo_small_lml_result {
    double terms[kSmallLmlTerms];
    int info, seq;
};
size_t small_lml_scratch_doubles();
void launch_small_lml(hipStream_t s, const cbo_small_set &st, double *scratch, int *info, cbo_small_lml_result *out, int seq);
size_t mid_lml_scratch_doubles();
void launch_small_lml_batch(hipStream_t s, const cbo_small_set *sets, int n_models, double *scratch, int64_t stride,
                            int *info, cbo_small_lml_result *out, int seq);
struct cbo_small_loo_result {
    double sum;
    double mean[128], var[128], lpd[128];
    int info, seq;
};
size_t small_loo_scratch_doubles();
void launch_small_loo_batch(hipStream_t s, const cbo_small_set *sets, int n_models, double *scratch, int *info,
                            cbo_small_loo_result *out, int seq);
void launch_loo_identity_chunk(hipStream_t s, double *V, int64_t ldv, int64_t rows, int64_t cols, int64_t shift);
int loo_finish_blocks(int64_t n);
void launch_loo_finish(hipStream_t s, const double *c, const double *alpha, const double *y, int64_t n, double *mean_out,
                       double *var_out, double *lpd_out, double *partial, double *sum_out);
constexpr int kSmallTwoPhaseFromBlocks = 12;
constexpr int kEiKind = 0;
constexpr int kMesKind = 5;
constexpr int kPredictKind = 6;
struct cbo_small_aux {
    int64_t off, count;
};
struct SmallAux {
    const cbo_small_aux *per_set = nullptr;
    const double *data = nullptr;
    double *mean_out = nullptr, *var_out = nullptr;
};
void launch_small_sets(hipStream_t s, int kind, const cbo_small_set *sets, int n_sets, int blocks_per_set, double *scratch,
                       double *part_val, int64_t *part_idx, int *info, int *ticket, cbo_small_result *out, int seq,
                       const SmallAux &aux = SmallAux());
void launch_small_sets_con(hipStream_t s, const cbo_small_set *pairs, int n_pairs, int n_sets, int max_pairs,
                           int blocks_per_set, double *scratch, double *part_val, int64_t *part_idx, int *info, int *ticket,
                           cbo_small_result *out, int seq);

size_t hyper_avg_scratch_doubles(int blocks, int n_samples);
void launch_hyper_avg(hipStream_t s, const cbo_small_set &st, const double *craw, const double *hyper, int n_samples,
                      int n_ls, double *acq_out, int blocks, int schedule, double *scratch, double *part_val,
                      int64_t *part_idx, int *info, int *ticket, cbo_small_result *out, int seq);
struct HyperArgs {
    cbo_small_set st;
    const double *craw;
    const double *hyper;
    int n_samples, n_ls;
    double *acq_out;
};
struct HyperSet {
    HyperArgs a;
    int first, pad_;
};
size_t hyper_sets_scratch_doubles(int n_sets, int blocks_per_set, int total_samples, bool two_phase);
void launch_hyper_sets(hipStream_t s, const HyperSet *sets, int n_sets, int blocks_per_set, int total_samples, bool two_phase,
                       double *scratch, double *part_val, int64_t *part_idx, int *info, int *ticket, cbo_small_result *out,
                       int seq);
void launch_hyper_accumulate(hipStream_t s, double *sum, const double *acq, int64_t m, bool first, int n_blocks);
void launch_hyper_finish(hipStream_t s, const double *sum, int64_t m, int n_samples, double *acq_out, double *part_val,
                         int64_t *part_idx, int64_t index_offset, int n_blocks);

struct AcqParams {
    double variance, noise_var, y_best, ei_jitter, cost;
    int task, include_noise, want_ei;
    const double *y_best_dev = nullptr;
};
void launch_acq(hipStream_t s, const double *q, const double *mu, const double *pm, const double *pv, int64_t m,
                const AcqParams &p, double *mean_out, double *var_out, double *acq_out, double *part_val,
                int64_t *part_idx, int64_t index_offset, int n_blocks);
void launch_argmax_final(hipStream_t s, const double *part_val, const int64_t *part_idx, int n, double *best_val,
                         int64_t *best_idx, const int *status_src = nullptr, int *status_dst = nullptr);
int acq_blocks_for(int64_t m);
constexpr int kMesMaxSamples = 64;
struct MesParams {
    double variance, noise_var, cost;
    int k;
    double mins[kMesMaxSamples];
};
void launch_mes_acq(hipStream_t s, const double *q, const double *mu, const double *pm, const double *pv, int64_t m,
                    const MesParams &p, double *mean_out, double *var_out, double *acq_out, double *part_val,
                    int64_t *part_idx, int64_t index_offset, int n_blocks);
struct GumbelSet {
    const double *mean, *var;
    int64_t m;
};
void launch_gumbel_quantiles(hipStream_t s, const GumbelSet &one, const GumbelSet *table, int n_sets, double *out,
                             int64_t *status);
constexpr int kConMaxModels = CBO_MAX_CONSTRAINTS + 1;
struct ConModel {
    const double *q, *mu, *pm, *pv;
    double *out;
    double variance, noise_var;
    double value, jitter;
    int sense, pad_;
};
struct ConParams {
    ConModel mdl[kConMaxModels];
    double y_best, ei_jitter, cost;
    int n_models, has_objective, task, pad_;
};
void launch_constrained_acq(hipStream_t s, const ConParams &p, int64_t m, double *acq_out, double *part_val,
                            int64_t *part_idx, int64_t index_offset, int n_blocks);
void launch_pointwise_acq(hipStream_t s, int kind, const double *q, const double *mu, const double *pm, const double *pv,
                          int64_t m, const AcqParams &p, double *mean_out, double *var_out, double *acq_out,
                          double *part_val, int64_t *part_idx, int64_t index_offset, int n_blocks);
void launch_plugin_incumbent(hipStream_t s, const double *mean, int64_t n, int task, double *out);
void launch_group_mean(hipStream_t s, const double *in, int64_t n_groups, int64_t group, double *out);

void launch_lml_terms(hipStream_t s, const double *A, int64_t lda, int64_t n_pad, const double *z, double *out2);
int lml_grad_tiles(int64_t n_pad);
void launch_lml_grad(hipStream_t s, const PointSet &X, const KernelHyper &h, const double *alpha, const double *negW,
                     int64_t ldw, int64_t n_pad, double *partial, double *out);
void launch_set_identity(hipStream_t s, double *V, int64_t ldv, int64_t n_pad);
void launch_gather_diag(hipStream_t s, const double *A, int64_t lda, int64_t n, double *diag);
void launch_export_lower(hipStream_t s, const double *A, int64_t lda, int64_t n, double *L_rowmajor);
void launch_export_sym(hipStream_t s, const double *A, int64_t lda, int64_t n, double *K_rowmajor);

int run_mfma_selftest(hipStream_t s, double *max_err);

void launch_append_commit(hipStream_t s, double *A, int64_t lda, int64_t n, int64_t n_pad, const double *l_src,
                          int64_t ld_src, double d, double zn, double *z, double *lvec, PointSet &X, const PointSet &P,
                          double pm_new, double pv_new, double *y, double y_new, double *invDt);
int append_row_slices(int64_t n);
void launch_append_row(hipStream_t s, double *V, int64_t ldv, int64_t n, const double *lvec, int64_t m_pad,
                       const double *krow, double d, double zn, double *partial, double *q, double *mu);

constexpr int kAppendLd = 64;
constexpr int kAppendMaxSlices = 8;
void launch_append_forward(hipStream_t s, const double *A, int64_t lda, int64_t n_pad, const double *invDt, double *W,
                           int64_t ldw, int kp, double *out);
struct AppendSchurArgs {
    const double *part; int slices;
    int k;
    const double *Kbb; int64_t ldk;
    const double *pv, *pm;
    const double *y_new;
    double variance, sigma;
    double *L22, *zb;
    int *status;
};
int append_schur_slices(int64_t n);
void launch_append_schur(hipStream_t s, const double *B, int64_t n, const double *z, AppendSchurArgs a);
struct AppendCommitArgs {
    double *A; int64_t lda, n, n_pad; int k;
    const double *B, *L22, *zb, *y_new;
    double *z, *y;
    int dims; double *xs; int64_t ldx; double *sq, *sv, *pm, *pv;
    const double *pxs; int64_t ldp; const double *psq, *psv, *pm_new, *pv_new;
};
// ... 56 lines not shown
```

cbo_with_oop_amd/csrc/kernels_chol.hip:

```cpp
#include <hip/hip_ext.h>
#include <climits>
#include <atomic>
#include <cstring>
#include <vector>

#include "cbo_small_device.h"

namespace cbo {

__global__ __launch_bounds__(256) void potrf_diag128_v2_kernel(double *A, int64_t lda, int r0, int rcol,
                                                               double *__restrict__ invDt, int *info,
                                                               double *__restrict__ zvec)
{
    extern __shared__ __align__(16) unsigned char smem_raw[];
    Diag2Shared &sh = *reinterpret_cast<Diag2Shared *>(smem_raw);
    if (__builtin_nontemporal_load(info) != 0) return;
    const int tid = threadIdx.x;
    const int lane = tid & 63;
    const int wave = __builtin_amdgcn_readfirstlane(tid >> 6);
    {
        const unsigned s0 = lds_byte_address(&sh.S[0][0]);
        const double *g = A + (int64_t)(r0 + wave * 32) * lda + r0 + lane * 2;
#pragma unroll 8
        for (int p = 0; p < 32; ++p) {
// ... 829 lines not shown
    const int nt = n2 / 64;
    if (ti_end > nt) ti_end = nt;
    if (ti_end <= ti_begin) return;
    hipLaunchKernelGGL(syrk_kernel<64>, dim3(nt + 1, ti_end - ti_begin), dim3(256), 0, s, A, lda, r0, n1, c0, nt, rcol,
                       ti_begin, skip_if);
}

static hipEvent_t event_slot(std::vector<hipEvent_t> &ev, size_t i)
{
    while (ev.size() <= i) {
        hipEvent_t e;
        hipEventCreateWithFlags(&e, hipEventDisableTiming | hipEventDisableSystemFence);
        ev.push_back(e);
    }
    return ev[i];
}

void sweep_pipe_pair(const SweepPipe &pipe, hipStream_t chain, const double *A, int64_t lda, const double *invDt,
                     int64_t n_pad, int p, int r0, int klen)
{
    auto pipe_event = [&](int kind, int pp) {
        return event_slot(*pipe.events, (size_t)(3 * pp + kind));
    };
    const int64_t cols = (pipe.lower_tri && r0 + klen < pipe.m_pad) ? (int64_t)(r0 + klen) : pipe.m_pad;
    const double m = (double)cols;
    hipEventRecord(pipe_event(0, p), chain);
    hipStreamWaitEvent(pipe.stream, pipe_event(0, p), 0);
    if (pipe.mark) pipe.mark(pipe.user, pipe.stream, 1, (double)klen * (double)klen * m);
    launch_trsm_strips(pipe.stream, A + (int64_t)r0 * lda + r0, lda, invDt + (int64_t)(r0 / 16) * 256,
                       pipe.V + (int64_t)r0 * pipe.ldv, pipe.ldv, klen, cols, pipe.zvec + r0, pipe.q, pipe.mu, true, true);
    if (pipe.mark) pipe.mark(pipe.user, pipe.stream, 0, 0.0);
    hipEventRecord(pipe_event(1, p), pipe.stream);
    const int below = r0 + klen;
    if (below >= (int)n_pad) return;
    const int first_end = (below + 256 < (int)n_pad) ? below + 256 : (int)n_pad;
    auto update = [&](hipStream_t st, int k0, int kl, int i0, int i1) {
        if (i0 >= i1) return;
        if (pipe.mark) pipe.mark(pipe.user, st, 1, 2.0 * (double)kl * (double)(i1 - i0) * m);
        launch_gemm_update(st, A, lda, pipe.V, pipe.ldv, pipe.V, pipe.ldv, k0, kl, i0, i1, cols, false);
        if (pipe.mark) pipe.mark(pipe.user, st, 0, 0.0);
    };
    const int G = pipe.group, lead = pipe.lead;
    const int full_pairs = ((pipe.tail_begin < (int)n_pad) ? pipe.tail_begin : (int)n_pad) / 256;
    const bool grouped = G >= 2 && !pipe.lower_tri && klen == 256 && p >= lead && ((p - lead) / G + 1) * G + lead <= full_pairs;
    if (grouped) {
        const int j = (p - lead) / G, i = (p - lead) % G;
        const int g0 = 256 * (lead + G * j);
        const int next_end = (g0 + 512 * G < (int)n_pad) ? g0 + 512 * G : (int)n_pad;
        if (i == 0 && j == 0 && lead > 0) hipStreamWaitEvent(pipe.stream, pipe_event(2, lead - 1), 0);
        update(pipe.stream, r0, 256, below, first_end);
        if (i == 0 && j >= 1) hipStreamWaitEvent(pipe.stream, pipe_event(2, lead + G * (j - 1)), 0);
        update(pipe.stream, r0, 256, r0 + 512, next_end);
        if (i < G - 1) return;
        hipStreamWaitEvent(pipe.bulk, pipe_event(1, p), 0);
        const int a1 = (g0 + 768 * G < (int)n_pad) ? g0 + 768 * G : (int)n_pad;
        update(pipe.bulk, g0, 256 * G, next_end, a1);
        hipEventRecord(pipe_event(2, lead + G * j), pipe.bulk);
        update(pipe.bulk, g0, 256 * G, a1, (int)n_pad);
        hipEventRecord(pipe_event(2, p), pipe.bulk);
        return;
    }
    if (p > 0) hipStreamWaitEvent(pipe.stream, pipe_event(2, p - 1), 0);
    update(pipe.stream, r0, klen, below, first_end);
    hipStreamWaitEvent(pipe.bulk, pipe_event(1, p), 0);
    update(pipe.bulk, r0, klen, first_end, (int)n_pad);
    hipEventRecord(pipe_event(2, p), pipe.bulk);
}

void sweep_pipe_tail(const SweepPipe &pipe, hipStream_t chain, const double *A, int64_t lda, const double *invDt,
                     int64_t n_pad, int pairs_done)
{
    std::vector<hipEvent_t> &ev = *pipe.events;
    const hipEvent_t last = event_slot(ev, (size_t)(3 * pairs_done));
    if (pairs_done > 0) {
        hipEventRecord(last, pipe.stream);
        hipStreamWaitEvent(chain, last, 0);
        hipStreamWaitEvent(chain, ev[(size_t)(3 * (pairs_done - 1) + 2)], 0);
    }
    const int t0 = pipe.tail_begin;
    const double rows = (double)((int)n_pad - t0);
    if (pipe.mark) pipe.mark(pipe.user, chain, 1, rows * rows * (double)pipe.m_pad);
    launch_trsm_strips(chain, A + (int64_t)t0 * lda + t0, lda, invDt + (int64_t)(t0 / 16) * 256,
                       pipe.V + (int64_t)t0 * pipe.ldv, pipe.ldv, (int64_t)n_pad - t0, pipe.m_pad, pipe.zvec + t0, pipe.q,
                       pipe.mu, true, false);
    if (pipe.mark) pipe.mark(pipe.user, chain, 0, 0.0);
}

__global__ void zero_ints_kernel(int *p, int n)
{
    for (int i = threadIdx.x; i < n; i += blockDim.x) p[i] = 0;
}

void launch_cholesky(hipStream_t s, hipStream_t side, std::vector<hipEvent_t> &events, double *A, int64_t lda,
                     int64_t n_pad, double *invDt, int *info_dev, const CholOptions &opt, const SweepPipe *pipe,
                     bool info_zeroed)
{
    hipFuncSetAttribute(reinterpret_cast<const void *>(potrf_diag128_v2_kernel), hipFuncAttributeMaxDynamicSharedMemorySize,
                        (int)sizeof(Diag2Shared));
    hipFuncSetAttribute(reinterpret_cast<const void *>(panel_trsm_kernel), hipFuncAttributeMaxDynamicSharedMemorySize,
                        (int)sizeof(PanelShared));
    hipFuncSetAttribute(reinterpret_cast<const void *>(potrf_panel_fused_kernel), hipFuncAttributeMaxDynamicSharedMemorySize,
                        (int)sizeof(Diag2Shared));
    constexpr int syrk_gemm_rows = 6144;
    auto launch_diag = [&](int rr) {
        hipLaunchKernelGGL(potrf_diag128_v2_kernel, dim3(1), dim3(256), sizeof(Diag2Shared), s, A, lda, rr, (int)n_pad,
                           invDt, info_dev, pipe ? pipe->zvec : nullptr);
    };
    const int np = (int)(n_pad / 128);
    const bool fused = opt.panel_form != 2 && 2 * np <= kCholFlagSlots;
    const bool split = opt.panel_form == 5;
    if (!info_zeroed) hipLaunchKernelGGL(zero_ints_kernel, dim3(1), dim3(256), 0, s, info_dev, fused ? 1 + 2 * np : 1);
    int *flags = info_dev + 1;
    const int rcol = (int)n_pad;
    event_slot(events, (size_t)(2 * np + 1));
    hipEventRecord(events[2 * np], s);
    hipStreamWaitEvent(side, events[2 * np], 0);
    double *zvec = pipe ? pipe->zvec : nullptr;
    const bool lean_panel = !pipe;
    int pair = 0;
    auto sweep_rows = [&](int r0, int klen) {
        if (pipe && r0 < pipe->tail_begin) sweep_pipe_pair(*pipe, s, A, lda, invDt, n_pad, pair++, r0, klen);
    };
    int pending = -1;
    int group_left = 0;
    int group_pairs = 0, group_g0 = 0, group_first_k = 0;
    int pending_big_a = -1;
    for (int k = 0; k < np; k += 2) {
        const int r0 = 128 * k;
        const int n2 = (int)n_pad - r0 - 128;
        const int n3_pair = (int)n_pad - r0 - 256;
        if (group_left == 0 && opt.bulk_group >= 2 && (fused || lean_panel)) {
            int G = 0;
            if (opt.bulk_group >= 4 && n3_pair - 1024 >= opt.group4_rows && n3_pair - 1024 >= syrk_gemm_rows &&
                n3_pair - 1024 >= 1024)
                G = 4;
            else if (n3_pair - 512 >= syrk_gemm_rows && n3_pair - 512 >= 512) G = 2;
            if (G != 0) { group_pairs = G; group_left = G; group_g0 = r0; group_first_k = k; }
        }
        const bool grouped = group_left > 0;
        const bool first_of_group = grouped && group_left == group_pairs;
        const bool last_of_group = grouped && group_left == 1;
        const bool split_now = split || grouped;
        auto factor_panel = [&](int r, int cols, hipEvent_t done) {
            if (fused && cols > 0) {
                launch_panel_fused(s, A, lda, r, rcol, invDt, info_dev, zvec, cols, flags + 2 * (r / 128), opt.spin_limit,
                                   done, split_now);
                return;
            }
            launch_diag(r);
            if (cols <= 0) return;
            if (lean_panel) launch_panel_trsm(s, A, lda, r, r + 128, cols, invDt, info_dev, done);
            else
                launch_trsm_strips(s, A + (int64_t)r * lda + r, lda, invDt + (int64_t)(r / 16) * 256,
                                   A + (int64_t)r * lda + r + 128, lda, 128, cols, nullptr, nullptr, nullptr, false, true);
        };
        factor_panel(r0, n2, nullptr);
        if (n2 <= 0) { sweep_rows(r0, 128); break; }
        launch_syrk_rows(s, A, lda, r0, 128, n2, rcol, info_dev);
        const int r1 = r0 + 128;
        const int n3 = (int)n_pad - r1 - 128;
        const bool bulk = n3 > 256;
        const bool gemm_form = bulk && n3 - 256 >= syrk_gemm_rows;
        const bool carried = bulk && (fused || lean_panel);
        const hipEvent_t ev_panel = (carried && gemm_form && (!grouped || last_of_group)) ? events[2 * k] : nullptr;
        const hipEvent_t ev_rows = (carried && !gemm_form) ? events[2 * k] : nullptr;
        factor_panel(r1, n3, ev_panel);
        sweep_rows(r0, 256);
        if (n3 <= 0) break;
        if (grouped) {
            const int S = 256 * group_pairs, g0 = group_g0, n = (int)n_pad;
            const int next_end = (g0 + 2 * S < n) ? g0 + 2 * S : n;
            if (last_of_group) {
                hipStreamWaitEvent(side, events[2 * k], 0);
                const int a_end = (g0 + 3 * S < n) ? g0 + 3 * S : n;
                launch_gemm_update(side, A, lda, A, lda, A, lda, g0, S, next_end, a_end, n_pad + kRhsCols, true, info_dev);
                hipEventRecord(events[2 * group_first_k + 1], side);
                pending_big_a = 2 * group_first_k + 1;
                if (a_end < n)
                    launch_gemm_update(side, A, lda, A, lda, A, lda, g0, S, a_end, n, n_pad + kRhsCols, true, info_dev);
                hipEventRecord(events[2 * k + 1], side);
                pending = 2 * k + 1;
            }
            launch_syrk_rows(s, A, lda, r0, 256, n3, rcol, info_dev, 256, nullptr);
            if (first_of_group && pending_big_a >= 0) hipStreamWaitEvent(s, events[pending_big_a], 0);
            launch_gemm_update(s, A, lda, A, lda, A, lda, r0, 256, r0 + 512, next_end, n_pad + kRhsCols, true, info_dev);
            --group_left;
            continue;
        }
        const int prev = pending;
        auto launch_bulk = [&] {
            if (!carried) hipEventRecord(events[2 * k], s);
            hipStreamWaitEvent(side, events[2 * k], 0);
            if (gemm_form)
                launch_gemm_update(side, A, lda, A, lda, A, lda, r0, 256, r0 + 256 + 256, (int)n_pad, n_pad + kRhsCols, true,
                                   info_dev);
            else
                launch_syrk(side, A, lda, r0, 256, n3, rcol, 4, n3 / 64, info_dev);
            hipEventRecord(events[2 * k + 1], side);
            pending = 2 * k + 1;
        };
        if (gemm_form) launch_bulk();
        if (prev >= 0) hipStreamWaitEvent(s, events[prev], 0);
        launch_syrk_rows(s, A, lda, r0, 256, n3, rcol, info_dev, 256, ev_rows);
        if (bulk && !gemm_form) launch_bulk();
    }
    hipEventRecord(events[2 * np + 1], side);
    hipStreamWaitEvent(s, events[2 * np + 1], 0);
    if (pipe && pipe->tail_begin < (int)n_pad) sweep_pipe_tail(*pipe, s, A, lda, invDt, n_pad, pair);
}

__global__ __launch_bounds__(256) void backsolve_step_kernel(const double *__restrict__ A, int64_t lda,
                                                             const double *__restrict__ invDt, int blk, double *zt,
                                                             double *__restrict__ alpha)
{
    __shared__ double zs[128];
    __shared__ double al[128];
    const int tid = threadIdx.x;
    const int lane = tid & 63, wave = tid >> 6;
    const int b0 = blk * 128;
    if (tid < 128) zs[tid] = zt[b0 + tid];
    __syncthreads();
    for (int s = 7; s >= 0; --s) {
        const int o = 16 * s;
        if (tid < 64) {
            const int i = tid >> 2, part = tid & 3;
            const double *Y = invDt + (int64_t)(b0 / 16 + s) * 256;
            double acc = 0.0;
#pragma unroll
            for (int k = 0; k < 4; ++k) acc = fma(Y[i * 16 + 4 * part + k], zs[o + 4 * part + k], acc);
            acc += __shfl_xor(acc, 1);
            acc += __shfl_xor(acc, 2);
            if (part == 0) al[o + i] = acc;
        }
        __syncthreads();
        if (tid < o) {
            const double *row = A + (int64_t)(b0 + tid) * lda + b0 + o;
            double acc = zs[tid];
#pragma unroll
            for (int c = 0; c < 16; ++c) acc = fma(-row[c], al[o + c], acc);
            zs[tid] = acc;
// ... 300 lines not shown
```

cbo_with_oop_amd/csrc/kernels_kmat.hip:

```cpp
#include "cbo_device.h"

#pragma clang fp contract(off)

namespace cbo {

__global__ __launch_bounds__(256) void prep_points_kernel(const double *__restrict__ raw, int64_t n, int d,
                                                          const double *__restrict__ ls,
                                                          const double *__restrict__ pv,
                                                          double *__restrict__ xs, int64_t ld,
                                                          double *__restrict__ sq, double *__restrict__ sv)
{
    const int64_t i = (int64_t)blockIdx.x * blockDim.x + threadIdx.x;
    if (i >= ld) return;
    double x[CBO_MAX_DIM];
#pragma unroll
    for (int k = 0; k < CBO_MAX_DIM; ++k) x[k] = 0.0;
    if (i < n) {
#pragma unroll
        for (int k = 0; k < CBO_MAX_DIM; ++k)
            if (k < d) {
                double v = raw[i * d + k];
                if (ls) v = v / ls[k];
                x[k] = v;
            }
    }
#pragma unroll
    for (int k = 0; k < CBO_MAX_DIM; ++k)
        if (k < d) xs[(int64_t)k * ld + i] = x[k];
    double s;
    if (d == 8) {
        double r[8];
#pragma unroll
        for (int k = 0; k < 8; ++k) r[k] = __dmul_rn(x[k], x[k]);
        s = __dadd_rn(__dadd_rn(__dadd_rn(r[0], r[1]), __dadd_rn(r[2], r[3])),
                      __dadd_rn(__dadd_rn(r[4], r[5]), __dadd_rn(r[6], r[7])));
    } else {
        s = 0.0;
#pragma unroll
        for (int k = 0; k < CBO_MAX_DIM; ++k)
            if (k < d) s = __dadd_rn(s, __dmul_rn(x[k], x[k]));
    }
    sq[i] = s;
    if (sv) sv[i] = (i < n && pv) ? sqrt(pv[i]) : 0.0;
}

__global__ __launch_bounds__(256) void prep_points_staged_kernel(const double *__restrict__ stage, int64_t n, int d,
                                                                 const double *__restrict__ ls, int has_prior,
                                                                 double *__restrict__ raw, double *__restrict__ y,
                                                                 double *__restrict__ pm, double *__restrict__ pv,
                                                                 double *__restrict__ xs, int64_t ld,
                                                                 double *__restrict__ sq, double *__restrict__ sv)
{
    const int64_t i = (int64_t)blockIdx.x * blockDim.x + threadIdx.x;
    if (i >= ld) return;
    double x[CBO_MAX_DIM];
#pragma unroll
    for (int k = 0; k < CBO_MAX_DIM; ++k) x[k] = 0.0;
    double pvi = 0.0;
    if (i < n) {
#pragma unroll
        for (int k = 0; k < CBO_MAX_DIM; ++k)
            if (k < d) {
                double v = stage[i * d + k];
                raw[i * d + k] = v;
                if (ls) v = v / ls[k];
                x[k] = v;
            }
        y[i] = stage[n * d + i];
        if (has_prior) {
            pm[i] = stage[n * d + n + i];
            pvi = stage[n * d + 2 * n + i];
            pv[i] = pvi;
        }
    }
#pragma unroll
    for (int k = 0; k < CBO_MAX_DIM; ++k)
        if (k < d) xs[(int64_t)k * ld + i] = x[k];
    double s;
    if (d == 8) {
        double r[8];
#pragma unroll
        for (int k = 0; k < 8; ++k) r[k] = __dmul_rn(x[k], x[k]);
        s = __dadd_rn(__dadd_rn(__dadd_rn(r[0], r[1]), __dadd_rn(r[2], r[3])),
                      __dadd_rn(__dadd_rn(r[4], r[5]), __dadd_rn(r[6], r[7])));
    } else {
        s = 0.0;
#pragma unroll
        for (int k = 0; k < CBO_MAX_DIM; ++k)
            if (k < d) s = __dadd_rn(s, __dmul_rn(x[k], x[k]));
    }
    sq[i] = s;
    if (sv) sv[i] = (i < n && has_prior) ? sqrt(pvi) : 0.0;
}

void launch_prep_points_staged(hipStream_t s, const double *stage, int64_t n, int d, const double *ls_dev, bool has_prior,
                               double *raw, double *y, double *pm, double *pv, double *xs, int64_t ld, double *sq,
                               double *sv)
{
    hipLaunchKernelGGL(prep_points_staged_kernel, dim3((unsigned)((ld + 255) / 256)), dim3(256), 0, s, stage, n, d, ls_dev,
                       has_prior ? 1 : 0, raw, y, pm, pv, xs, ld, sq, sv);
}

void launch_prep_points(hipStream_t s, const double *raw_aos, int64_t n, int d, const double *ls_dev,
                        const double *pv_raw, double *xs, int64_t ld, double *sq, double *sv)
{
    const int threads = 256;
    const int blocks = (int)((ld + threads - 1) / threads);
    hipLaunchKernelGGL(prep_points_kernel, dim3(blocks), dim3(threads), 0, s, raw_aos, n, d, ls_dev, pv_raw, xs, ld,
                       sq, sv);
}

struct KmatArgs {
    const double *rx; int64_t ldr; const double *rsq; const double *rsv;
    const double *cx; int64_t ldc; const double *csq; const double *csv;
    int64_t n_rows, n_cols;
    int64_t col_begin;
    double *out; int64_t ldo;
    double variance, lengthscale, diag_add, jitter;
    int symmetric, zero_diag;
    int sym_tiles;
    float *out32;
    const double *alpha;
    double *mu_part;
    int64_t ld_part;
};

template <int D, bool OUT32 = false>
__global__ __launch_bounds__(256) void kmat_tile_kernel(KmatArgs a)
{
    int tj = blockIdx.x, ti = blockIdx.y;
    if (a.symmetric) {
        const int nt = a.sym_tiles;
        const int t = blockIdx.x;
        ti = (int)((2.0 * nt + 1.0 - sqrt((2.0 * nt + 1.0) * (2.0 * nt + 1.0) - 8.0 * (double)t)) * 0.5);
        while (ti > 0 && ti * nt - ti * (ti - 1) / 2 > t) --ti;
        while ((ti + 1) * nt - (ti + 1) * ti / 2 <= t) ++ti;
        tj = ti + (t - (ti * nt - ti * (ti - 1) / 2));
    }
    __shared__ double sx[D][64], sy[D][64];
    __shared__ double sxq[64], syq[64], sxv[64], syv[64];
    __shared__ double sal[OUT32 ? 64 : 1], smu[OUT32 ? 8 * 64 : 1];
    const int tid = threadIdx.x;
    const int64_t i0 = (int64_t)ti * 64, j0 = (int64_t)tj * 64;
    if (OUT32 && tid >= 128 && tid < 192) {
        const int64_t gi = i0 + (tid - 128);
        sal[tid - 128] = (gi < a.n_rows) ? a.alpha[gi] : 0.0;
    }
    double macc[2] = {0.0, 0.0};
    if (tid < 64) {
        const int64_t gi = i0 + tid;
        const bool in = gi < a.ldr;
#pragma unroll
        for (int k = 0; k < D; ++k) sx[k][tid] = in ? a.rx[(int64_t)k * a.ldr + gi] : 0.0;
        sxq[tid] = in ? a.rsq[gi] : 0.0;
        sxv[tid] = (in && a.rsv) ? a.rsv[gi] : 0.0;
    } else if (tid < 128) {
        const int t = tid - 64;
        const int64_t gj = a.col_begin + j0 + t;
#pragma unroll
        for (int k = 0; k < D; ++k) sy[k][t] = a.cx[(int64_t)k * a.ldc + gj];
        syq[t] = a.csq[gj];
        syv[t] = a.csv ? a.csv[gj] : 0.0;
    }
    __syncthreads();
    const int tx = tid & 31, ty = tid >> 5;
    const bool causal = (a.rsv != nullptr) && (a.csv != nullptr);
    const double inv_l2 = 1.0 / (a.lengthscale * a.lengthscale);
    double yj[2][D];
#pragma unroll
    for (int c = 0; c < 2; ++c)
#pragma unroll
        for (int k = 0; k < D; ++k) yj[c][k] = sy[k][2 * tx + c];
#pragma unroll
    for (int rr = 0; rr < 8; ++rr) {
        const int ii = ty + 8 * rr;
        const int64_t gi = i0 + ii;
        double xi[D];
#pragma unroll
        for (int k = 0; k < D; ++k) xi[k] = sx[k][ii];
        d2 o;
#pragma unroll
        for (int c = 0; c < 2; ++c) {
            const int jj = 2 * tx + c;
            const int64_t gj = j0 + jj;
            const bool row_ok = gi < a.n_rows;
            const bool col_ok = (a.col_begin + gj) < a.n_cols;
            double v;
            if (a.symmetric) {
                if (row_ok && col_ok) {
                    v = kernel_value<D>(xi, yj[c], sxq[ii], syq[jj], a.variance, inv_l2,
                                        a.zero_diag && gi == gj);
                    if (causal) v = __dadd_rn(v, __dmul_rn(sxv[ii], syv[jj]));
                    if (gi == gj) {
                        v = __dadd_rn(v, a.diag_add);
                        if (a.jitter != 0.0) v = __dadd_rn(v, a.jitter);
                    }
                } else {
                    v = (gi == gj) ? 1.0 : 0.0;
                }
            } else {
                if (row_ok) {
                    v = kernel_value<D>(xi, yj[c], sxq[ii], syq[jj], a.variance, inv_l2, false);
                    if (causal) v = __dadd_rn(v, __dmul_rn(sxv[ii], syv[jj]));
                } else {
                    v = 0.0;
                }
            }
            o[c] = v;
        }
        if (OUT32) {
            macc[0] = __fma_rn(o[0], sal[ii], macc[0]);
            macc[1] = __fma_rn(o[1], sal[ii], macc[1]);
            const int64_t pr = (gi & ~(int64_t)15) + 4 * (gi & 3) + ((gi >> 2) & 3);
            typedef float f2 __attribute__((ext_vector_type(2)));
            f2 of;
            of[0] = (float)o[0];
            of[1] = (float)o[1];
            *reinterpret_cast<f2 *>(&a.out32[pr * a.ldo + j0 + 2 * tx]) = of;
        } else {
            *reinterpret_cast<d2 *>(&a.out[gi * a.ldo + j0 + 2 * tx]) = o;
        }
    }
    if (OUT32) {
        smu[ty * 64 + 2 * tx] = macc[0];
        smu[ty * 64 + 2 * tx + 1] = macc[1];
        __syncthreads();
        if (tid < 64) {
            double t = 0.0;
#pragma unroll
            for (int g = 0; g < 8; ++g) t = __dadd_rn(t, smu[g * 64 + tid]);
            a.mu_part[(int64_t)ti * a.ld_part + j0 + tid] = t;
        }
    }
}

template <int D>
static void launch_kmat_d(hipStream_t s, const KmatArgs &a, dim3 grid)
{
    if (a.out32) hipLaunchKernelGGL((kmat_tile_kernel<D, true>), grid, dim3(256), 0, s, a);
    else hipLaunchKernelGGL((kmat_tile_kernel<D, false>), grid, dim3(256), 0, s, a);
}

static void launch_kmat(hipStream_t s, int d, const KmatArgs &a, dim3 grid)
{
    switch (d) {
        case 1: launch_kmat_d<1>(s, a, grid); break;
        case 2: launch_kmat_d<2>(s, a, grid); break;
        case 3: launch_kmat_d<3>(s, a, grid); break;
        case 4: launch_kmat_d<4>(s, a, grid); break;
        case 5: launch_kmat_d<5>(s, a, grid); break;
        case 6: launch_kmat_d<6>(s, a, grid); break;
        case 7: launch_kmat_d<7>(s, a, grid); break;
        default: launch_kmat_d<8>(s, a, grid); break;
    }
}

void launch_kxx(hipStream_t s, const PointSet &X, const KernelHyper &h, double diag_add, double jitter, double *A,
                int64_t lda, int64_t n_pad)
{
    KmatArgs a;
    a.rx = X.xs; a.ldr = X.ld; a.rsq = X.sq; a.rsv = X.sv;
    a.cx = X.xs; a.ldc = X.ld; a.csq = X.sq; a.csv = X.sv;
    a.n_rows = X.n; a.n_cols = X.n; a.col_begin = 0;
    a.out = A; a.ldo = lda;
    a.variance = h.variance; a.lengthscale = h.lengthscale; a.diag_add = diag_add; a.jitter = jitter;
    a.symmetric = 1; a.zero_diag = h.zero_diag; a.out32 = nullptr; a.alpha = nullptr; a.mu_part = nullptr; a.ld_part = 0;
    const int nt = (int)(n_pad / 64);
    a.sym_tiles = nt;
    launch_kmat(s, X.d, a, dim3((unsigned)(nt * (nt + 1) / 2), 1));
}

void launch_kstar(hipStream_t s, const PointSet &X, const PointSet &C, int64_t c_begin, int64_t m_pad,
                  const KernelHyper &h, double *V, int64_t ldv, int64_t n_pad)
{
    KmatArgs a;
    a.rx = X.xs; a.ldr = X.ld; a.rsq = X.sq; a.rsv = X.sv;
    a.cx = C.xs; a.ldc = C.ld; a.csq = C.sq; a.csv = (X.sv != nullptr) ? C.sv : nullptr;
    a.n_rows = X.n; a.n_cols = C.ld; a.col_begin = c_begin;
    a.out = V; a.ldo = ldv;
    a.variance = h.variance; a.lengthscale = h.lengthscale; a.diag_add = 0.0; a.jitter = 0.0;
    a.symmetric = 0; a.zero_diag = 0; a.sym_tiles = 0; a.out32 = nullptr; a.alpha = nullptr; a.mu_part = nullptr; a.ld_part = 0;
    launch_kmat(s, X.d, a, dim3((unsigned)(m_pad / 64), (unsigned)(n_pad / 64)));
}

__global__ __launch_bounds__(256) void colsum_parts_kernel(const double *__restrict__ part, int64_t ld, int tiles,
                                                           int64_t m, double *__restrict__ mu)
{
    const int64_t c = (int64_t)blockIdx.x * 256 + threadIdx.x;
    if (c >= m) return;
    double t = 0.0;
    for (int i = 0; i < tiles; ++i) t = __dadd_rn(t, part[(int64_t)i * ld + c]);
    mu[c] = t;
}

void launch_kstar_f32(hipStream_t s, const PointSet &X, const PointSet &C, int64_t c_begin, int64_t m_pad,
                      const KernelHyper &h, float *V, int64_t ldv, int64_t n32, const double *alpha, double *mu_part,
                      double *mu)
{
    KmatArgs a;
    a.rx = X.xs; a.ldr = X.ld; a.rsq = X.sq; a.rsv = X.sv;
    a.cx = C.xs; a.ldc = C.ld; a.csq = C.sq; a.csv = (X.sv != nullptr) ? C.sv : nullptr;
    a.n_rows = X.n; a.n_cols = C.ld; a.col_begin = c_begin;
    a.out = nullptr; a.ldo = ldv; a.out32 = V;
    a.alpha = alpha; a.mu_part = mu_part; a.ld_part = m_pad;
    a.variance = h.variance; a.lengthscale = h.lengthscale; a.diag_add = 0.0; a.jitter = 0.0;
    a.symmetric = 0; a.zero_diag = 0; a.sym_tiles = 0;
    launch_kmat(s, X.d, a, dim3((unsigned)(m_pad / 64), (unsigned)(n32 / 64)));
    hipLaunchKernelGGL(colsum_parts_kernel, dim3((unsigned)((m_pad + 255) / 256)), dim3(256), 0, s, mu_part, m_pad,
                       (int)(n32 / 64), m_pad, mu);
}

__global__ __launch_bounds__(256) void rhs_kernel(const double *__restrict__ y, const double *__restrict__ pm,
                                                  int64_t n, double *__restrict__ A, int64_t lda, int64_t n_pad,
                                                  int *__restrict__ zero, int zero_count)
{
    if (blockIdx.x == 0)
        for (int i = threadIdx.x; i < zero_count; i += blockDim.x) zero[i] = 0;
    const int64_t idx = (int64_t)blockIdx.x * blockDim.x + threadIdx.x;
    if (idx >= n_pad * kRhsCols) return;
    const int64_t i = idx / kRhsCols;
    const int c = (int)(idx % kRhsCols);
    double v = 0.0;
    if (c == 0 && i < n) v = pm ? __dadd_rn(y[i], -pm[i]) : y[i];
    A[i * lda + n_pad + c] = v;
}

void launch_rhs(hipStream_t s, const double *y, const double *pm, int64_t n, double *A, int64_t lda, int64_t n_pad,
                int *zero, int zero_count)
{
    const int64_t total = n_pad * kRhsCols;
    hipLaunchKernelGGL(rhs_kernel, dim3((unsigned)((total + 255) / 256)), dim3(256), 0, s, y, pm, n, A, lda, n_pad, zero,
                       zero ? zero_count : 0);
}

__global__ __launch_bounds__(256) void zero_pair_kernel(double *__restrict__ a, double *__restrict__ b, int64_t n)
{
    const int64_t i = (int64_t)blockIdx.x * blockDim.x + threadIdx.x;
    if (i < n) { a[i] = 0.0; b[i] = 0.0; }
}

void launch_zero_pair(hipStream_t s, double *a, double *b, int64_t n)
{
    if (n > 0) hipLaunchKernelGGL(zero_pair_kernel, dim3((unsigned)((n + 255) / 256)), dim3(256), 0, s, a, b, n);
}

__global__ void gather_diag_kernel(const double *__restrict__ A, int64_t lda, int64_t n, double *__restrict__ diag)
{
    const int64_t i = (int64_t)blockIdx.x * blockDim.x + threadIdx.x;
    if (i < n) diag[i] = A[i * lda + i];
}

void launch_gather_diag(hipStream_t s, const double *A, int64_t lda, int64_t n, double *diag)
{
    hipLaunchKernelGGL(gather_diag_kernel, dim3((unsigned)((n + 255) / 256)), dim3(256), 0, s, A, lda, n, diag);
}

__global__ __launch_bounds__(256) void lml_terms_kernel(const double *__restrict__ A, int64_t lda, int64_t n_pad,
                                                        const double *__restrict__ z, double *__restrict__ out2)
{
    __shared__ double s1[256], s2[256];
    double a = 0.0, b = 0.0;
    for (int64_t i = threadIdx.x; i < n_pad; i += 256) {
        const double zi = z[i];
        a = __fma_rn(zi, zi, a);
        b = __dadd_rn(b, log(A[i * lda + i]));
    }
    s1[threadIdx.x] = a;
    s2[threadIdx.x] = b;
    __syncthreads();
    for (int st = 128; st > 0; st >>= 1) {
        if ((int)threadIdx.x < st) {
            s1[threadIdx.x] = __dadd_rn(s1[threadIdx.x], s1[threadIdx.x + st]);
            s2[threadIdx.x] = __dadd_rn(s2[threadIdx.x], s2[threadIdx.x + st]);
        }
        __syncthreads();
    }
    if (threadIdx.x == 0) { out2[0] = s1[0]; out2[1] = s2[0]; }
}

void launch_lml_terms(hipStream_t s, const double *A, int64_t lda, int64_t n_pad, const double *z, double *out2)
{
    hipLaunchKernelGGL(lml_terms_kernel, dim3(1), dim3(256), 0, s, A, lda, n_pad, z, out2);
}

template <int D>
__global__ __launch_bounds__(256) void lml_grad_tile_kernel(const double *__restrict__ xs, int64_t ldx, int64_t n,
                                                            const double *__restrict__ alpha,
                                                            const double *__restrict__ negW, int64_t ldw,
                                                            double variance, double inv_l2_iso,
                                                            const double *__restrict__ sv ,
                                                            double *__restrict__ partial )
{
    const int tj = blockIdx.x, ti = blockIdx.y;
    const int tile = ti * gridDim.x + tj;
    __shared__ double sx[D][64], sy[D][64], sa[64], sb[64], svx[64], svy[64];
    __shared__ double red[256];
    const int tid = threadIdx.x;
    double s[1 + D];
#pragma unroll
    for (int k = 0; k <= D; ++k) s[k] = 0.0;
    if (tj >= ti) {
        const int64_t i0 = (int64_t)ti * 64, j0 = (int64_t)tj * 64;
        if (tid < 64) {
#pragma unroll
            for (int k = 0; k < D; ++k) sx[k][tid] = xs[(int64_t)k * ldx + i0 + tid];
            sa[tid] = (i0 + tid < n) ? alpha[i0 + tid] : 0.0;
            svx[tid] = (sv && i0 + tid < n) ? sv[i0 + tid] : 0.0;
        } else if (tid < 128) {
            const int t = tid - 64;
#pragma unroll
            for (int k = 0; k < D; ++k) sy[k][t] = xs[(int64_t)k * ldx + j0 + t];
            sb[t] = (j0 + t < n) ? alpha[j0 + t] : 0.0;
            svy[t] = (sv && j0 + t < n) ? sv[j0 + t] : 0.0;
        }
        __syncthreads();
// ... 224 lines not shown
```

cbo_with_oop_amd/csrc/kernels_trsm.hip:

```cpp
#include <cstdlib>
#include <type_traits>

#include "cbo_internal.h"

namespace cbo {

#define MFMA_F64(a, b, c) __builtin_amdgcn_mfma_f64_16x16x4f64((a), (b), (c), 0, 0, 0)

#define SCHED_DS(n) __builtin_amdgcn_sched_group_barrier(0x100, (n), 0)
#define SCHED_MFMA(n) __builtin_amdgcn_sched_group_barrier(0x008, (n), 0)
#define SCHED_VMEM(n) __builtin_amdgcn_sched_group_barrier(0x010, (n), 0)

constexpr int kRB = 128;
constexpr int kT = kRB / 16;
constexpr int kLdsLd = kRB + 16;
constexpr int kNBuf = 3;
template <int KB>
struct StageGeom {
    static constexpr int kA = KB * kLdsLd;
    static constexpr int kB = 4 * KB * 16;
    static constexpr int kRA = KB / 4;
    static constexpr int kParts = KB / 8;
    static constexpr int kDma = 3 * kParts;
    static constexpr int kKS = KB / 4;
    static constexpr int kDiagStages = kRB / KB;
    static constexpr int kDiagTiles = KB / 16;
    static constexpr int kDiagStores = 4 * kDiagTiles;
    static_assert(kParts <= kKS - 2, "the DMA groups and the cursor update ride under the first k-steps");
};

struct StageCursor {
    int i0, j, lim;
    int ai0, aj;
    const double *a_src;
    const double *b_src;
    int64_t b_stride;
};

template <bool SWEEP, int KB>
__global__ __launch_bounds__(256) void trsm_strip_kernel(const double *__restrict__ U, int64_t ldu,
                                                         const double *__restrict__ invDt, double *V, int64_t ldv,
                                                         int n, const double *__restrict__ z,
                                                         double *__restrict__ q_out, double *__restrict__ mu_out,
                                                         int accumulate)
{
    using G = StageGeom<KB>;
    constexpr int kKB = KB, kABuf = G::kA, kBBuf = G::kB, kDmaPerStage = G::kDma, kStoresPerDiagStage = G::kDiagStores;
    constexpr int kDS = G::kDiagStages, kDT = G::kDiagTiles, kKS = G::kKS, kParts = G::kParts;
    __shared__ __align__(16) double lds[kNBuf * (kABuf + kBBuf)];

    const int tid = threadIdx.x;
    const int lane = tid & 63;
    const int wave = __builtin_amdgcn_readfirstlane(tid >> 6);
    const int lc = lane & 15, kq = lane >> 4;
    const int64_t colw = (int64_t)blockIdx.x * kStrip + wave * 16;
    double *Vc = V + colw + lc;
    double *ldsB = lds + kNBuf * kABuf;
    const unsigned lds_byte0 = lds_byte_address(lds);
    const double *ug = U + (int64_t)(wave * G::kRA) * ldu + lane * 2;
    const double *vg = V + (int64_t)(lane >> 3) * ldv + colw + 2 * (lane & 7);

    const double *inv_lane = invDt + lane * 2;
    auto locate_a = [&](StageCursor &c) __attribute__((always_inline)) {
        const bool past = c.i0 >= n;
        c.ai0 = past ? n - kRB : c.i0;
        c.aj = past ? (n - kRB) / kKB + kDS - 1 : c.j;
    };
    auto locate_b = [&](StageCursor &c) __attribute__((always_inline)) {
        c.a_src = ug + (int64_t)(kKB * c.aj) * ldu + c.ai0;
    };
    auto locate_c = [&](StageCursor &c) __attribute__((always_inline)) {
        const int nreg = c.ai0 / kKB;
        const int64_t diag = (c.aj >= nreg) ? 1 : 0;
        const int64_t off_diag = ((int64_t)(c.ai0 / 16) + kDT * (c.aj - nreg)) * 256;
        const int64_t off_reg = (int64_t)(kKB * c.aj) * ldv;
        const uintptr_t base = (uintptr_t)vg + ((uintptr_t)inv_lane - (uintptr_t)vg) * (uintptr_t)diag;
        c.b_src = reinterpret_cast<const double *>(base) + (off_reg + (off_diag - off_reg) * diag);
        c.b_stride = 8 * ldv + (128 - 8 * ldv) * diag;
    };
    auto locate = [&](StageCursor &c) __attribute__((always_inline)) {
        locate_a(c);
        locate_b(c);
        locate_c(c);
    };
    auto step = [&](StageCursor &c) __attribute__((always_inline)) {
        const int wrap = (c.j + 1 == c.lim) ? 1 : 0;
// ... 551 lines not shown
                        hand[1] = macc;
                        qacc = 0.0;
                        macc = 0.0;
                    } else if (((i0 / kRB) & 1) || i0 + kRB >= n) {
                        qacc += __shfl_xor(qacc, 16);
                        qacc += __shfl_xor(qacc, 32);
                        macc += __shfl_xor(macc, 16);
                        macc += __shfl_xor(macc, 32);
                        qtot += qacc;
                        mtot += macc;
                        qacc = 0.0;
                        macc = 0.0;
                    } else {
                        hand[0] = qacc;
                        hand[1] = macc;
                    }
                }
            } else if (hs == 0) {
                double uf[kDT][kTH][4], xb[kDT][4];
#pragma unroll
                for (int hh = 0; hh < kDT; ++hh)
#pragma unroll
                    for (int t = 0; t < kTH; ++t)
#pragma unroll
                        for (int kk = 0; kk < 4; ++kk)
                            uf[hh][t][kk] = abase0[(16 * hh + 4 * kk) * kLdsLd + 16 * (kTH + t)];
                stage_dma();
#pragma unroll
                for (int hh = 0; hh < kDT; ++hh) {
                    asm volatile("s_waitcnt lgkmcnt(0)" ::: "memory");
                    __builtin_amdgcn_s_barrier();
#pragma unroll
                    for (int kk = 0; kk < 4; ++kk) xb[hh][kk] = xreg[hh * 256 + (4 * kk + kq) * 16 + lc];
#pragma unroll
                    for (int kk = 0; kk < 4; ++kk)
#pragma unroll
                        for (int t = 0; t < kTH; ++t) acc[t] = MFMA_F64(uf[hh][t][kk], xb[hh][kk], acc[t]);
                }
            } else {
                stage_dma();
            }
            buf = (buf == 2) ? 0 : buf + 1;
        }
#pragma unroll
        for (int t = 0; t < kTH; ++t)
#pragma unroll
            for (int r = 0; r < 4; ++r) {
                asm volatile("" : "+v"(accn[t][r]));
                acc[t][r] = -accn[t][r];
            }
        if (SWEEP) {
            asm volatile("" : "+v"(zn));
            *reinterpret_cast<d2 *>(zl + (((i0 / kRB) + 1) & 1) * kRB + 2 * lane) = zn;
        }
    }
#undef STAGE8_TOP
    asm volatile("s_waitcnt vmcnt(0)" ::: "memory");
    __builtin_amdgcn_s_barrier();

    if (SWEEP && h == 1 && kq == 0) {
        q_out[colw + lc] = qtot;
        mu_out[colw + lc] = mtot;
    }
}

constexpr int kPB = 2 * kRB;
constexpr int kPKB = 16;
constexpr int kPLd = kPB + 16;
constexpr int kPA = kPKB * kPLd;
constexpr int kPBd = 4 * kPKB * 16;
constexpr int kPDma = 5;
constexpr int kPD0 = kRB / 16;
constexpr int kPD1 = kRB / 32;

struct PairCursor {
    int i0, j, lim;
    int ai0, aj;
    const double *a_src;
    int64_t a_cstride;
    const double *b_src;
    unsigned b_dst;
};

template <bool SWEEP>
__global__ __launch_bounds__(512) void trsm_pair_kernel(const double *__restrict__ U, int64_t ldu,
                                                        const double *__restrict__ invDt, double *V, int64_t ldv,
                                                        int n, const double *__restrict__ z,
                                                        double *__restrict__ q_out, double *__restrict__ mu_out,
                                                        int accumulate)
{
    __shared__ __align__(16) double lds[kNBuf * (kPA + kPBd)];
    __shared__ __align__(16) double zl[SWEEP ? 2 * kPB : 2];
    __shared__ __align__(16) double handbuf[SWEEP ? 4 * 64 * 2 : 2];

    const int tid = threadIdx.x;
    const int lane = tid & 63;
    const int wave = __builtin_amdgcn_readfirstlane(tid >> 6);
    const int cw = wave & 3, h = wave >> 2;
    const int lc = lane & 15, kq = lane >> 4;
    const int64_t colw = (int64_t)blockIdx.x * kStrip + cw * 16;
    double *Vq = V + colw + lc + (int64_t)kq * ldv;
    double *ldsB = lds + kNBuf * kPA;
    double *hand = handbuf + (cw * 64 + lane) * 2;
    const unsigned lds_byte0 = lds_byte_address(lds);
    const double *ug = U + (int64_t)(2 * wave) * ldu + lane * 2;
    const double *vg = V + (int64_t)((lane >> 3) + 8 * h) * ldv + colw + 2 * (lane & 7);
    const double *inv_d0 = invDt + 128 * h + lane * 2;
    const double *inv_d1 = invDt + 256 * (cw >> 1) + 128 * (cw & 1) + lane * 2;

    PairCursor ahead{0, 0, kPD0 + kPD1, 0, 0, nullptr, 0, nullptr, 0u};
    auto locate_a = [&](PairCursor &c) __attribute__((always_inline)) {
        const bool past = c.i0 >= n;
        c.ai0 = past ? n - kPB : c.i0;
        c.aj = past ? (n - kPB) / kPKB + kPD0 + kPD1 - 1 : c.j;
    };
    auto locate_b = [&](PairCursor &c) __attribute__((always_inline)) {
        const int m1 = c.aj - c.ai0 / kPKB - kPD0;
        const bool d1 = m1 >= 0;
        const int64_t row = d1 ? (int64_t)(c.ai0 + kRB + 32 * m1) : (int64_t)kPKB * c.aj;
        const int64_t col = d1 ? (int64_t)(c.ai0 + kRB) : (int64_t)c.ai0;
        c.a_src = ug + row * ldu + col;
        c.a_cstride = d1 ? 16 * ldu : (int64_t)kRB;
    };
    auto locate_c = [&](PairCursor &c) __attribute__((always_inline)) {
        const int nreg = c.ai0 / kPKB;
        const int m1 = c.aj - nreg - kPD0;
        const bool d1 = m1 >= 0, reg = c.aj < nreg;
        const int64_t tile = d1 ? (int64_t)(nreg + kPD0 + 2 * m1) : (int64_t)c.aj;
        const double *inv_p = (d1 ? inv_d1 : inv_d0) + tile * 256;
        const double *v_p = vg + (int64_t)(kPKB * c.aj) * ldv;
        c.b_src = reg ? v_p : inv_p;
        c.b_dst = d1 ? (unsigned)(cw * 128) : (unsigned)(cw * 256 + 128 * h);
    };
    auto step = [&](PairCursor &c) __attribute__((always_inline)) {
        const int wrap = (c.j + 1 == c.lim) ? 1 : 0;
        c.i0 += kPB * wrap;
        c.j = (c.j + 1) * (1 - wrap);
        c.lim = c.lim + (c.i0 / kPKB + kPD0 + kPD1 - c.lim) * wrap;
    };
    auto advance = [&](PairCursor &c) __attribute__((always_inline)) {
        step(c);
        locate_a(c);
        locate_b(c);
        locate_c(c);
    };
    auto issue_one = [&](const PairCursor &c, int buf, int i) __attribute__((always_inline)) {
        if (i < 4) {
            const unsigned la = __builtin_amdgcn_readfirstlane(
                lds_byte0 + 8u * (unsigned)(buf * kPA + (2 * wave + (i >> 1)) * kPLd + kRB * (i & 1)));
            glds16(c.a_src + (int64_t)(i >> 1) * ldu + (int64_t)(i & 1) * c.a_cstride, la);
        } else {
            const unsigned lb = __builtin_amdgcn_readfirstlane(lds_byte0 + 8u * ((unsigned)(kNBuf * kPA + buf * kPBd) + c.b_dst));
            glds16(c.b_src, lb);
        }
    };
    auto issue_stage = [&](const PairCursor &c, int buf) __attribute__((always_inline)) {
#pragma unroll
        for (int i = 0; i < kPDma; ++i) issue_one(c, buf, i);
    };

    auto run = [&](auto role_tag) __attribute__((always_inline)) {
        constexpr int H = decltype(role_tag)::value;
        d4 acc[kT];
#pragma unroll
        for (int t = 0; t < kT; ++t)
#pragma unroll
            for (int r = 0; r < 4; ++r) acc[t][r] = -Vq[(int64_t)(kRB * H + 16 * t + 4 * r) * ldv];
        if (SWEEP) {
            const d2 z0 = *reinterpret_cast<const d2 *>(z + kRB * H + 2 * lane);
            *reinterpret_cast<d2 *>(zl + kRB * H + 2 * lane) = z0;
        }
        double accn[kT][4];
        d2 zn;
        constexpr int kAhead = kT * 4 + (SWEEP ? 1 : 0);
        const unsigned vq_off = (unsigned)(((int64_t)kq * ldv + lc) * 8);
        const unsigned z_off = (unsigned)(lane * 16);
        constexpr int kL0 = 16, kL1 = kAhead - kL0;
        auto request_one = [&](int i0, int sl) __attribute__((always_inline)) {
            const int nb = (i0 + kPB < n) ? i0 + kPB : i0;
            const double *vb = V + colw + (int64_t)(nb + kRB * H) * ldv;
            if (sl < kT * 4)
                asm volatile("global_load_dwordx2 %0, %1, %2" : "=v"(accn[sl >> 2][sl & 3]) : "v"(vq_off), "s"(vb + (int64_t)(4 * sl) * ldv) : "memory");
            else if (SWEEP)
                asm volatile("global_load_dwordx4 %0, %1, %2" : "=v"(zn) : "v"(z_off), "s"(z + nb + kRB * H) : "memory");
        };

        locate_a(ahead);
        locate_b(ahead);
        locate_c(ahead);
        issue_stage(ahead, 0);
        advance(ahead);
        issue_stage(ahead, 1);
        advance(ahead);

        int buf = 0;
        double qacc = 0.0, macc = 0.0, qtot = 0.0, mtot = 0.0;
        if (SWEEP && accumulate && H == 1) {
            qtot = q_out[colw + lc];
            mtot = mu_out[colw + lc];
        }

        int a1 = 0, b1 = 0, a2 = 0;
        auto wait_top = [&]() __attribute__((always_inline)) {
            asm volatile("s_waitcnt lgkmcnt(0)" ::: "memory");
            const int extra = a1 + b1 + a2;
#define WAIT_IF(x) if (extra == (x)) asm volatile("s_waitcnt vmcnt(%0)" ::"n"(kPDma + (x)) : "memory")
            if (extra == 0) asm volatile("s_waitcnt vmcnt(%0)" ::"n"(kPDma) : "memory");
            else WAIT_IF(4);
            else WAIT_IF(8);
            else WAIT_IF(16);
            else WAIT_IF(kL1);
            else WAIT_IF(kL0 + 4);
            else WAIT_IF(kL0 + 8);
            else WAIT_IF(kL0 + kL1);
            else WAIT_IF(kL1 + 16);
            else WAIT_IF(kL0 + kL1 + 16);
            else asm volatile("s_waitcnt vmcnt(%0)" ::"n"(kPDma) : "memory");
#undef WAIT_IF
            __builtin_amdgcn_s_barrier();
            __builtin_amdgcn_sched_barrier(0);
            a2 = a1;
            a1 = 0;
            b1 = 0;
        };
        static_assert(kPDma + kL0 + kL1 + 16 <= 63 && kL1 >= kL0, "s_waitcnt vmcnt is a 6-bit count; the cases of wait_top");

        double af[2][kT], bf[2];
        auto regular_stage = [&](int i0, auto first_tag) __attribute__((always_inline)) {
            constexpr bool FIRST = decltype(first_tag)::value;
            const int zpar = ((i0 / kPB) & 1) * kPB;
            wait_top();
            if (FIRST) {
#pragma unroll
                for (int t = 0; t < kT; ++t)
#pragma unroll
                    for (int r = 0; r < 4; ++r) {
                        asm volatile("; ahead-pin %0" : "+v"(accn[t][r]));
                        acc[t][r] = -accn[t][r];
                    }
                if (SWEEP) {
                    asm volatile("; ahead-pin %0" : "+v"(zn));
                    *reinterpret_cast<d2 *>(zl + zpar + kRB * H + 2 * lane) = zn;
                }
// ... 197 lines not shown
                            for (int r = 0; r < 4; ++r) zr[hh][r] = zl[zpar + kRB + 16 * (s + hh) + kq + 4 * r];
                    }
                    __builtin_amdgcn_sched_barrier(0);
                    x += x2;
                    asm volatile("" : "+v"(x));
                    auto emit = [&](int hh, const d4 &xx) __attribute__((always_inline)) {
#pragma unroll
                        for (int r = 0; r < 4; ++r) {
                            asm volatile("global_store_dwordx2 %0, %1, %2" ::"v"(vq_off), "v"(xx[r]), "s"(V + colw + (int64_t)(i0 + kRB + 16 * (s + hh) + 4 * r) * ldv) : "memory");
                            if (SWEEP) {
                                qacc = fma(xx[r], xx[r], qacc);
                                macc = fma(xx[r], zr[hh][r], macc);
                            }
                        }
                        if (SWEEP) asm volatile("" : "+v"(qacc), "+v"(macc));
                    };
#pragma unroll
                    for (int kk = 0; kk < 4; ++kk) {
                        acc[s + 1] = MFMA_F64(uf[0][s + 1][kk], x[kk], acc[s + 1]);
                        if (s + 2 < kT) acc[s + 2] = MFMA_F64(uf[0][s + 2][kk], x[kk], acc[s + 2]);
                        __builtin_amdgcn_sched_barrier(0);
                        if (kk == 0) { issue_one(ahead, bnext, 0); issue_one(ahead, bnext, 1); }
                        else if (kk == 1) { issue_one(ahead, bnext, 2); issue_one(ahead, bnext, 3); }
                        else if (kk == 2) issue_one(ahead, bnext, 4);
                        else advance(ahead);
                        __builtin_amdgcn_sched_barrier(0);
                    }
                    emit(0, x);
                    const d4 na = -acc[s + 1];
                    d4 y1 = {0.0, 0.0, 0.0, 0.0}, y2 = {0.0, 0.0, 0.0, 0.0};
#pragma unroll
                    for (int kk = 0; kk < 4; ++kk) {
                        if (kk & 1) y2 = MFMA_F64(iv[1][kk], na[kk], y2);
                        else y1 = MFMA_F64(iv[1][kk], na[kk], y1);
#pragma unroll
                        for (int t = s + 3; t < kT; ++t) {
                            acc[t] = MFMA_F64(uf[0][t][kk], x[kk], acc[t]);
                            if (SWEEP && m == 1 && kk == 0 && t == s + 3) request_one(i0, kT * 4);
                        }
                    }
#pragma unroll
                    for (int t = s + 2; t < kT; ++t)
#pragma unroll
                        for (int kk = 0; kk < 4; ++kk) uf[1][t][kk] = ab[(4 * kk) * kPLd + kRB + 16 * t];
                    const d4 y = y1 + y2;
                    emit(1, y);
#pragma unroll
                    for (int kk = 0; kk < 4; ++kk)
#pragma unroll
                        for (int t = s + 2; t < kT; ++t) {
                            acc[t] = MFMA_F64(uf[1][t][kk], y[kk], acc[t]);
                            const int idx = kk * (kT - s - 2) + (t - s - 2);
                            if (m < 2 && idx < 16) request_one(i0, 16 * m + idx);
                        }
                    a1 += 8 + (m == 0 ? kL0 : m == 1 ? kL1 : 0);
                    if (SWEEP && m == kPD1 - 1) {
                        qacc += __shfl_xor(qacc, 16);
                        qacc += __shfl_xor(qacc, 32);
                        macc += __shfl_xor(macc, 16);
                        macc += __shfl_xor(macc, 32);
                        qtot += qacc;
                        mtot += macc;
                        qacc = 0.0;
                        macc = 0.0;
                    }
                    buf = (buf == 2) ? 0 : buf + 1;
                }
            }
        };
        diag_phase(0, std::true_type{});
        for (int i0 = kPB; i0 < n; i0 += kPB) {
            const int nst = i0 / kPKB;
            regular_stage(i0, std::true_type{});
            for (int j = 1; j < nst; ++j) regular_stage(i0, std::false_type{});
            diag_phase(i0, std::false_type{});
        }
        asm volatile("s_waitcnt vmcnt(0)" ::: "memory");
        __builtin_amdgcn_s_barrier();

        if (SWEEP && H == 1 && kq == 0) {
            q_out[colw + lc] = qtot;
            mu_out[colw + lc] = mtot;
        }
    };
    if (h == 0) run(std::integral_constant<int, 0>{});
    else run(std::integral_constant<int, 1>{});
}

constexpr int kAccMoves = kT * 4;

template <int KB>
__global__ __launch_bounds__(256) void trsm_update_kernel(const double *__restrict__ U, int64_t ldu,
                                                          const double *V, int64_t ldv, double *C, int64_t ldc, int k0,
                                                          int klen, int i0_begin, int i0_end, int chunk_rows,
                                                          int upper_only, const int *__restrict__ skip_if)
{
    if (skip_if && __builtin_nontemporal_load(skip_if) != 0) return;
    using G = StageGeom<KB>;
    constexpr int kA = G::kA, kB = G::kB, kRA = G::kRA, kParts = G::kParts, kDma = G::kDma, kKS = G::kKS;
    __shared__ __align__(16) double lds[kNBuf * (kA + kB)];

    const int tid = threadIdx.x;
    const int lane = tid & 63;
    const int wave = __builtin_amdgcn_readfirstlane(tid >> 6);
    const int lc = lane & 15, kq = lane >> 4;
    const int64_t colw = (int64_t)blockIdx.x * kStrip + wave * 16;
    const int ib = i0_begin + (int)blockIdx.y * chunk_rows;
    const int ie = (ib + chunk_rows < i0_end) ? ib + chunk_rows : i0_end;
    if (ib >= ie) return;
    if (upper_only && (int)blockIdx.x * kStrip + kStrip <= ib) return;
    const int nst = klen / KB;
    double *Cc = C + colw + lc;
    double *ldsB = lds + kNBuf * kA;
    const unsigned lds_byte0 = lds_byte_address(lds);
    const double *ug = U + (int64_t)(k0 + wave * kRA) * ldu + lane * 2;
    const double *vg = V + (int64_t)(k0 + (lane >> 3)) * ldv + colw + 2 * (lane & 7);
    const int64_t b_stride = 8 * ldv;

    int ci0 = ib, cj = 0;
    const double *a_src, *b_src;
    auto locate = [&]() __attribute__((always_inline)) {
        const bool past = ci0 >= ie;
        const int ai0 = past ? ie - kRB : ci0;
        const int aj = past ? nst - 1 : cj;
        a_src = ug + (int64_t)(KB * aj) * ldu + ai0;
        b_src = vg + (int64_t)(KB * aj) * ldv;
    };
    auto advance = [&]() __attribute__((always_inline)) {
        const int wrap = (cj + 1 == nst) ? 1 : 0;
        ci0 += kRB * wrap;
        cj = (cj + 1) * (1 - wrap);
        locate();
    };
    auto issue_one = [&](int buf, int part, int q) __attribute__((always_inline)) {
        if (q < 2) {
            const unsigned la = __builtin_amdgcn_readfirstlane(lds_byte0 + 8u * (unsigned)(buf * kA + (wave * kRA) * kLdsLd));
            const int p = 2 * part + q;
            glds16(a_src + (int64_t)p * ldu, la + 8u * (unsigned)(p * kLdsLd));
        } else {
            const unsigned lb = __builtin_amdgcn_readfirstlane(
                lds_byte0 + 8u * (unsigned)(kNBuf * kA + buf * kB + wave * (KB * 16)));
            glds16(b_src + part * b_stride, lb + 8u * (unsigned)(part * 128));
        }
    };
    auto issue_part = [&](int buf, int part) __attribute__((always_inline)) {
#pragma unroll
        for (int q = 0; q < 3; ++q) issue_one(buf, part, q);
    };

    d4 acc[kT], accn[kT];
#pragma unroll
    for (int t = 0; t < kT; ++t)
#pragma unroll
        for (int r = 0; r < 4; ++r) acc[t][r] = -Cc[(int64_t)(ib + 16 * t + kq + 4 * r) * ldc];

    locate();
#pragma unroll
    for (int part = 0; part < kParts; ++part) issue_part(0, part);
    advance();
#pragma unroll
    for (int part = 0; part < kParts; ++part) issue_part(1, part);
    advance();

    int buf = 0;
    int boundary = 0;
    for (int i0 = ib; i0 < ie; i0 += kRB) {
        double af[2][kT], bf[2];
        bool deferred = false;
        for (int j = 0; j < nst; ++j) {
            asm volatile("s_waitcnt lgkmcnt(0)" ::: "memory");
            if (boundary) asm volatile("s_waitcnt vmcnt(%0)" ::"n"(kDma + kAccMoves) : "memory");
            else asm volatile("s_waitcnt vmcnt(%0)" ::"n"(kDma) : "memory");
            __builtin_amdgcn_s_barrier();
            boundary = (boundary > 0) ? boundary - 1 : 0;
            if (j == 0 && i0 + kRB < ie) {
#pragma unroll
                for (int t = 0; t < kT; ++t)
#pragma unroll
                    for (int r = 0; r < 4; ++r) accn[t][r] = -Cc[(int64_t)(i0 + kRB + 16 * t + kq + 4 * r) * ldc];
                asm volatile("" ::: "memory");
            }
            __builtin_amdgcn_sched_barrier(0);
            const int bnext = (buf >= 1) ? buf - 1 : 2;
            const double *abase = lds + buf * kA + kq * kLdsLd + lc;
            const double *bbase = ldsB + buf * kB + wave * (KB * 16) + kq * 16 + lc;
#pragma unroll
            for (int t = 0; t < kT; ++t) {
                if (deferred) acc[t] = MFMA_F64(af[1][t], bf[1], acc[t]);
                if (t < kT / 2) {
                    af[0][2 * t] = abase[32 * t];
                    af[0][2 * t + 1] = abase[32 * t + 16];
                } else if (t == kT / 2) {
                    bf[0] = bbase[0];
                }
                __builtin_amdgcn_sched_barrier(0);
            }
#pragma unroll
            for (int jj = 0; jj < kKS - 1; ++jj) {
                const double *an = abase + 4 * (jj + 1) * kLdsLd;
#pragma unroll
                for (int t = 0; t < kT; ++t) {
                    acc[t] = MFMA_F64(af[jj & 1][t], bf[jj & 1], acc[t]);
                    if (t < kT / 2) {
                        af[(jj + 1) & 1][2 * t] = an[32 * t];
                        af[(jj + 1) & 1][2 * t + 1] = an[32 * t + 16];
                    } else if (t == kT / 2) {
                        bf[(jj + 1) & 1] = bbase[4 * (jj + 1) * 16];
                    } else if (jj < kParts) {
                        issue_one(bnext, jj, t - (kT / 2 + 1));
                    } else if (jj == kParts && t == kT / 2 + 1) {
                        advance();
                    }
                    __builtin_amdgcn_sched_barrier(0);
                }
            }
            deferred = true;
            buf = (buf == 2) ? 0 : buf + 1;
        }
#pragma unroll
        for (int t = 0; t < kT; ++t) acc[t] = MFMA_F64(af[1][t], bf[1], acc[t]);
#pragma unroll
        for (int t = 0; t < kT; ++t)
#pragma unroll
            for (int r = 0; r < 4; ++r) Cc[(int64_t)(i0 + 16 * t + kq + 4 * r) * ldc] = -acc[t][r];
        asm volatile("" ::: "memory");
#pragma unroll
        for (int t = 0; t < kT; ++t) acc[t] = accn[t];
        boundary = 2;
    }
    asm volatile("s_waitcnt vmcnt(0)" ::: "memory");
    __builtin_amdgcn_s_barrier();
}

void launch_trsm_strips(hipStream_t s, const double *U, int64_t ldu, const double *invDt, double *V, int64_t ldv,
                        int64_t n, int64_t m_pad, const double *z, double *q, double *mu, bool accumulate,
                        bool half_lds)
{
    if (n <= 0 || m_pad <= 0) return;
    const dim3 grid((unsigned)(m_pad / kStrip));
    const int acc = accumulate ? 1 : 0;
    if (half_lds) {
        if (q != nullptr)
            hipLaunchKernelGGL((trsm_strip_kernel<true, 16>), grid, dim3(256), 0, s, U, ldu, invDt, V, ldv, (int)n, z, q, mu, acc);
        else
            hipLaunchKernelGGL((trsm_strip_kernel<false, 16>), grid, dim3(256), 0, s, U, ldu, invDt, V, ldv, (int)n, z, q, mu, 0);
        return;
    }
    static const bool pairs = [] {
        const char *e = getenv("CBO_HIP_STRIP_FORM");
        return !(e && atoi(e) == 8);
    }();
    if (pairs && n >= kPB && n % kPB == 0) {
        if (q != nullptr)
            hipLaunchKernelGGL((trsm_pair_kernel<true>), grid, dim3(512), 0, s, U, ldu, invDt, V, ldv, (int)n, z, q, mu, acc);
        else
            hipLaunchKernelGGL((trsm_pair_kernel<false>), grid, dim3(512), 0, s, U, ldu, invDt, V, ldv, (int)n, z, q, mu, 0);
        return;
    }
    if (q != nullptr)
        hipLaunchKernelGGL((trsm_strip8_kernel<true>), grid, dim3(512), 0, s, U, ldu, invDt, V, ldv, (int)n, z, q, mu, acc);
    else
        hipLaunchKernelGGL((trsm_strip8_kernel<false>), grid, dim3(512), 0, s, U, ldu, invDt, V, ldv, (int)n, z, q, mu, 0);
}

void launch_gemm_update(hipStream_t s, const double *U, int64_t ldu, const double *V, int64_t ldv, double *C,
                        int64_t ldc, int k0, int klen, int i0_begin, int i0_end, int64_t m_pad, bool upper_only,
                        const int *skip_if)
{
    if (i0_begin >= i0_end || m_pad <= 0 || klen <= 0) return;
    const dim3 grid((unsigned)(m_pad / kStrip), (unsigned)((i0_end - i0_begin + kRB - 1) / kRB));
    const int up = upper_only ? 1 : 0;
    hipLaunchKernelGGL(trsm_update_kernel<16>, grid, dim3(256), 0, s, U, ldu, V, ldv, C, ldc, k0, klen, i0_begin, i0_end, kRB,
                       up, skip_if);
}

__global__ void mfma_selftest_kernel(const double *A, const double *B, double *C)
{
    const int l = threadIdx.x;
    d4 acc = {0.0, 0.0, 0.0, 0.0};
    for (int k0 = 0; k0 < 16; k0 += 4)
        acc = MFMA_F64(A[(l & 15) * 16 + k0 + (l >> 4)], B[(k0 + (l >> 4)) * 16 + (l & 15)], acc);
    d4 acc2 = {0.0, 0.0, 0.0, 0.0};
    for (int kk = 0; kk < 4; ++kk) acc2 = MFMA_F64(A[(l & 15) * 16 + 4 * kk + (l >> 4)], acc[kk], acc2);
    for (int r = 0; r < 4; ++r) {
        C[((l >> 4) + 4 * r) * 16 + (l & 15)] = acc[r];
        C[256 + ((l >> 4) + 4 * r) * 16 + (l & 15)] = acc2[r];
    }
}

int run_mfma_selftest(hipStream_t s, double *max_err)
{
    double hA[256], hB[256], hC[512], ref[256], ref2[256];
    for (int i = 0; i < 16; ++i)
        for (int j = 0; j < 16; ++j) {
            hA[i * 16 + j] = (double)((i * 7 + j * 3) % 11 - 5);
            hB[i * 16 + j] = (double)((i * 5 + j * 13 + 1) % 17 - 8);
        }
    for (int i = 0; i < 16; ++i)
        for (int j = 0; j < 16; ++j) {
            double acc = 0.0;
            for (int k = 0; k < 16; ++k) acc += hA[i * 16 + k] * hB[k * 16 + j];
            ref[i * 16 + j] = acc;
        }
    for (int i = 0; i < 16; ++i)
        for (int j = 0; j < 16; ++j) {
            double acc = 0.0;
            for (int k = 0; k < 16; ++k) acc += hA[i * 16 + k] * ref[k * 16 + j];
            ref2[i * 16 + j] = acc;
        }
    double *dA = nullptr, *dB = nullptr, *dC = nullptr;
    if (hipMalloc(&dA, sizeof(hA)) != hipSuccess || hipMalloc(&dB, sizeof(hB)) != hipSuccess ||
        hipMalloc(&dC, sizeof(hC)) != hipSuccess)
        return -1;
    hipMemcpyAsync(dA, hA, sizeof(hA), hipMemcpyHostToDevice, s);
    hipMemcpyAsync(dB, hB, sizeof(hB), hipMemcpyHostToDevice, s);
    hipLaunchKernelGGL(mfma_selftest_kernel, dim3(1), dim3(64), 0, s, dA, dB, dC);
    hipMemcpyAsync(hC, dC, sizeof(hC), hipMemcpyDeviceToHost, s);
    const hipError_t e = hipStreamSynchronize(s);
    hipFree(dA); hipFree(dB); hipFree(dC);
    if (e != hipSuccess) return -1;
    double m = 0.0;
    for (int i = 0; i < 256; ++i) {
        const double e1 = fabs(hC[i] - ref[i]), e2 = fabs(hC[256 + i] - ref2[i]);
        if (e1 > m) m = e1;
        if (e2 > m) m = e2;
    }
    *max_err = m;
    return 0;
}

}
```

Baseline: 3.066 million.

## Fuse acquisition argmax finish into TRSM pair kernel and split Kxx assembly head

Adds a fused finish path where the last TRSM pair kernel computes posterior, acquisition and a per-strip argmax, then uses an atomic ticket so the last block reduces partials and writes the best value, index and status straight to pinned host memory. This removes the separate acquisition/reduction launch and the stream join events on the pipelined sweep path. It also splits Kxx assembly into a head kernel that builds the leading tiles together with the RHS, passing the remaining tiles to the Cholesky launcher so they can be deferred. The risks are ticket-reset correctness across calls and the extra register and LDS pressure in the TRSM kernel.

```diff
diff --git a/cbo_with_oop_amd/csrc/cbo_api.hip b/cbo_with_oop_amd/csrc/cbo_api.hip
--- a/cbo_with_oop_amd/csrc/cbo_api.hip
+++ b/cbo_with_oop_amd/csrc/cbo_api.hip
@@ -92,6 +92,10 @@
     int n_cu_pipe = 256;
     ScheduleTable schedule;
     int64_t fused_fallbacks = 0;
+    bool fused_finish = true;
+    int *fin_ticket = nullptr;
+    SweepFinish *h_fin = nullptr;
+    bool fit_head = true;
     bool sweep_cache = true;
     bool small_sets = true;
     int sweep_mode = -1;
@@ -361,6 +365,9 @@
     if (e == hipSuccess) e = hipEventCreateWithFlags(&c->ev_fork, hipEventDisableTiming | hipEventDisableSystemFence);
     if (e == hipSuccess) e = hipMalloc(&c->part_val, 2048 * sizeof(double));
     if (e == hipSuccess) e = hipMalloc(&c->part_idx, 2048 * sizeof(int64_t));
+    if (e == hipSuccess) e = hipMalloc(&c->fin_ticket, sizeof(int));
+    if (e == hipSuccess) e = hipMemset(c->fin_ticket, 0, sizeof(int));
+    if (e == hipSuccess) e = hipHostMalloc(&c->h_fin, sizeof(SweepFinish));
     if (e == hipSuccess) e = hipMalloc(&c->best_val, sizeof(double));
     if (e == hipSuccess) e = hipMalloc(&c->best_idx, sizeof(int64_t));
     if (e == hipSuccess) e = hipHostMalloc(&c->h_best_val, sizeof(double));
@@ -383,6 +390,10 @@
     if (hs) c->hyper_schedule = std::atoi(hs);
     const char *sc = std::getenv("CBO_HIP_SWEEP_CACHE");
     if (sc && std::atoi(sc) == 0) c->sweep_cache = false;
+    const char *ff = std::getenv("CBO_HIP_FUSED_FINISH");
+    if (ff && std::atoi(ff) == 0) c->fused_finish = false;
+    const char *fh = std::getenv("CBO_HIP_FIT_HEAD");
+    if (fh && std::atoi(fh) == 0) c->fit_head = false;
     const char *ss = std::getenv("CBO_HIP_SMALL_SETS");
     if (ss && std::atoi(ss) == 0) c->small_sets = false;
     const char *om = std::getenv("CBO_HIP_OVERLAP");
@@ -437,6 +448,8 @@
     if (c->stream) hipStreamSynchronize(c->stream);
     for (auto &p : c->pending) { hipEventDestroy(p.a); hipEventDestroy(p.b); }
     for (auto e : c->pool) hipEventDestroy(e);
+    hipFree(c->fin_ticket);
+    hipHostFree(c->h_fin);
     hipFree(c->part_val); hipFree(c->part_idx); hipFree(c->best_val); hipFree(c->best_idx);
     hipHostFree(c->h_best_val); hipHostFree(c->h_best_idx); hipHostFree(c->h_info); hipHostFree(c->stage);
     if (c->stage_done) hipEventDestroy(c->stage_done);
@@ -675,18 +688,31 @@
     return o;
 }
 
+static const KxxRest *enqueue_assembly(cbo_gp *g, double jitter, KxxRest *rest)
+{
+    cbo_ctx *c = g->ctx;
+    PhaseScope ps(c, PH_KXX);
+    const double diag_add = g->noise_var + kGpyDiagJitter;
+    if (!c->fit_head) {
+        launch_kxx(c->stream, g->X, g->h, diag_add, jitter, g->A, g->lda, g->n_pad);
+        launch_rhs(c->stream, g->y, g->X.pm, g->n, g->A, g->lda, g->n_pad, g->info, cholesky_info_ints(g->n_pad));
+        return nullptr;
+    }
+    launch_fit_head(c->stream, g->X, g->h, diag_add, jitter, g->A, g->lda, g->n_pad, g->y, g->info,
+                    cholesky_info_ints(g->n_pad));
+    *rest = KxxRest{&g->X, g->h, diag_add, jitter};
+    return rest;
+}
+
 static void enqueue_factor(cbo_gp *g, double jitter, bool separate)
 {
     cbo_ctx *c = g->ctx;
-    {
-        PhaseScope ps(c, PH_KXX);
-        launch_kxx(c->stream, g->X, g->h, g->noise_var + kGpyDiagJitter, jitter, g->A, g->lda, g->n_pad);
-        launch_rhs(c->stream, g->y, g->X.pm, g->n, g->A, g->lda, g->n_pad, g->info, cholesky_info_ints(g->n_pad));
-    }
+    KxxRest rest_store;
+    const KxxRest *rest = enqueue_assembly(g, jitter, &rest_store);
     {
         PhaseScope ps(c, PH_CHOL);
         launch_cholesky(c->stream, c->side_stream, c->chol_events, g->A, g->lda, g->n_pad, g->invDt, g->info,
-                        chol_options(c, separate), nullptr, true);
+                        chol_options(c, separate), nullptr, true, rest);
     }
 }
 
@@ -1203,8 +1229,41 @@
     return CBO_OK;
 }
 
+struct FusedFinish {
+    const SweepFinish *args = nullptr;
+    bool fused = false;
+};
+
+static bool fused_finish_wanted(const cbo_gp *g, const double *acq_out, const double *mean_out, const double *var_out,
+                                const MesParams *mes, int kind, const double *y_best_dev)
+{
+    return g->ctx->fused_finish && g->dtype != CBO_DTYPE_F32 && !acq_out && !mean_out && !var_out && !mes && kind == 0 &&
+           !y_best_dev;
+}
+
+static bool fused_finish_fits(int64_t rows, int64_t cols) { return sweep_finish_fusable(rows, cols); }
+
+static void fill_fused_finish(FusedFinish *f, const cbo_gp *g, const cbo_cands *k, double y_best, int task, double ei_jitter,
+                              double cost, bool with_status)
+{
+    cbo_ctx *c = g->ctx;
+    const bool causal = g->X.sv != nullptr;
+    SweepFinish &a = *c->h_fin;
+    f->args = c->h_fin;
+    a.p.variance = g->h.variance; a.p.noise_var = g->noise_var; a.p.y_best = y_best; a.p.ei_jitter = ei_jitter; a.p.cost = cost;
+    a.p.task = task; a.p.include_noise = 1; a.p.want_ei = 1;
+    a.p.y_best_dev = nullptr;
+    a.pm = causal ? k->pm : nullptr; a.pv = causal ? k->pv : nullptr;
+    a.m = k->m; a.index_offset = k->index_offset;
+    a.part_val = c->part_val; a.part_idx = c->part_idx; a.ticket = c->fin_ticket;
+    a.strips = (int)(k->m_pad / kStrip);
+    a.best_val = c->h_best_val; a.best_idx = c->h_best_idx;
+    a.status_src = with_status ? g->info : nullptr; a.status_dst = with_status ? c->h_info : nullptr;
+    f->fused = false;
+}
+
 static int solve_columns(cbo_gp *g, const cbo_cands *k, int64_t c_begin, int64_t cols, double *V, int64_t ldv, double *q,
-                         double *mu)
+                         double *mu, FusedFinish *fin = nullptr)
 {
     cbo_ctx *c = g->ctx;
     {
@@ -1212,10 +1271,13 @@
         launch_kstar(c->stream, g->X, k->P, c_begin, cols, g->h, V, ldv, g->n_pad);
     }
     if (prefer_right_looking(c, g->n_pad, cols)) return enqueue_right_looking(g, V, ldv, cols, q, mu);
+    const bool finish = fin && c_begin == 0 && cols == k->m_pad && fused_finish_fits(g->n_pad, cols);
     {
         PhaseScope ps(c, PH_TRSM);
-        launch_trsm_strips(c->stream, g->A, g->lda, g->invDt, V, ldv, g->n_pad, cols, g->z, q, mu);
-    }
+        launch_trsm_strips(c->stream, g->A, g->lda, g->invDt, V, ldv, g->n_pad, cols, g->z, q, mu, false, false,
+                           finish ? fin->args : nullptr);
+    }
+    if (finish) fin->fused = true;
     if (c->profiling) {
         c->timers.n_trsm_launches += 1;
         c->timers.trsm_flops += (double)g->n_pad * (double)g->n_pad * (double)cols;
@@ -1223,7 +1285,7 @@
     return CBO_OK;
 }
 
-static int enqueue_posterior(cbo_gp *g, cbo_cands *k, bool want_f64_solution = false)
+static int enqueue_posterior(cbo_gp *g, cbo_cands *k, bool want_f64_solution = false, FusedFinish *fin = nullptr)
 {
     cbo_ctx *c = g->ctx;
     int rc = prepare_cands(g, k);
@@ -1240,7 +1302,7 @@
     }
     for (int64_t c0 = 0; c0 < k->m_pad; c0 += chunk) {
         const int64_t cols = (k->m_pad - c0 < chunk) ? (k->m_pad - c0) : chunk;
-        rc = solve_columns(g, k, c0, cols, Vws, ldv, c->q + c0, c->mu + c0);
+        rc = solve_columns(g, k, c0, cols, Vws, ldv, c->q + c0, c->mu + c0, fin);
         if (rc != CBO_OK) return rc;
     }
     HIP_TRY(hipGetLastError());
@@ -1326,14 +1388,16 @@
 
 static int finish_sweep(cbo_gp *g, cbo_cands *k, double y_best, int task, double ei_jitter, double cost,
                         double *acq_out, double *mean_out, double *var_out, double *best_val, int64_t *best_idx,
-                        const MesParams *mes = nullptr, int kind = 0, const double *y_best_dev = nullptr)
+                        const MesParams *mes = nullptr, int kind = 0, const double *y_best_dev = nullptr,
+                        bool already_finished = false)
 {
     cbo_ctx *c = g->ctx;
     const double *q_src = nullptr, *mu_src = nullptr;
     int rc = settle_vectors(g, k, false, &q_src, &mu_src);
     if (rc != CBO_OK) return rc;
-    rc = enqueue_finish(g, k, y_best, task, ei_jitter, cost, acq_out, mean_out, var_out, q_src, mu_src, false, true, mes,
-                        kind, y_best_dev);
+    if (!already_finished)
+        rc = enqueue_finish(g, k, y_best, task, ei_jitter, cost, acq_out, mean_out, var_out, q_src, mu_src, false, true, mes,
+                            kind, y_best_dev);
     if (rc != CBO_OK) return rc;
     HIP_TRY(hipStreamSynchronize(c->stream));
     complete_finish(c, best_val, best_idx);
@@ -1594,7 +1658,7 @@
     return CBO_OK;
 }
 
-static int enqueue_vectors(cbo_gp *g, cbo_cands *k, bool *substituted = nullptr)
+static int enqueue_vectors(cbo_gp *g, cbo_cands *k, bool *substituted = nullptr, FusedFinish *fin = nullptr)
 {
     int rc = CBO_OK;
     cbo_ctx *c = g->ctx;
@@ -1606,7 +1670,7 @@
     if (!(c->sweep_cache && k->fit_stamp != 0 && k->fit_stamp == g->fit_stamp)) {
         k->fit_stamp = 0;
         if (substituted) *substituted = true;
-        return enqueue_posterior(g, k);
+        return enqueue_posterior(g, k, false, fin);
     }
     return grow_vectors(c, k->m_pad);
 }
@@ -1616,10 +1680,13 @@
                       int kind = 0, const double *y_best_dev = nullptr)
 {
     HIP_TRY(hipSetDevice(g->ctx->device));
-    const int rc = enqueue_vectors(g, k);
+    FusedFinish fin;
+    const bool want_fused = fused_finish_wanted(g, acq_out, mean_out, var_out, mes, kind, y_best_dev);
+    if (want_fused) fill_fused_finish(&fin, g, k, y_best, task, ei_jitter, cost, false);
+    const int rc = enqueue_vectors(g, k, nullptr, want_fused ? &fin : nullptr);
     if (rc != CBO_OK) return rc;
     return finish_sweep(g, k, y_best, task, ei_jitter, cost, acq_out, mean_out, var_out, best_val, best_idx, mes, kind,
-                        y_best_dev);
+                        y_best_dev, fin.fused);
 }
 
 extern "C" int cbo_acq_sweep(cbo_gp *g, cbo_cands *k, double y_best, int task, double ei_jitter, double cost,
@@ -1925,6 +1992,7 @@
     }
     const bool speculate = qbuf == k->q;
     SweepPipe pipe = make_pipe(g, Vws, ldv, k->m_pad, qbuf, mubuf);
+    FusedFinish fin;
     pipe.group = choice.group;
     int pairs = choice.pairs;
     pipe.lead = 0;
@@ -1932,17 +2000,20 @@
         pipe.lead = forced ? (c->pipe_lead > 0 ? c->pipe_lead : 0) : (c->pipe_lead >= 0 ? c->pipe_lead : pairs % pipe.group);
     pipe.tail_begin = pairs * 256;
     if (pipe.tail_begin > (int)g->n_pad) pipe.tail_begin = (int)g->n_pad;
+    if (speculate && fused_finish_wanted(g, acq_out, mean_out, var_out, nullptr, 0, nullptr) &&
+        fused_finish_fits(g->n_pad - pipe.tail_begin, k->m_pad)) {
+        fill_fused_finish(&fin, g, k, y_best, task, ei_jitter, cost, true);
+        fin.fused = true;
+        pipe.finish = fin.args;
+    }
     double jitter = 0.0;
     int tries = 0;
     bool separate = false;
     for (;;) {
         HIP_TRY(hipEventRecord(c->ev_fork, c->stream));
         HIP_TRY(hipStreamWaitEvent(c->sweep_stream, c->ev_fork, 0));
-        {
-            PhaseScope ps(c, PH_KXX);
-            launch_kxx(c->stream, g->X, g->h, g->noise_var + kGpyDiagJitter, jitter, g->A, g->lda, g->n_pad);
-            launch_rhs(c->stream, g->y, g->X.pm, g->n, g->A, g->lda, g->n_pad, g->info, cholesky_info_ints(g->n_pad));
-        }
+        KxxRest rest_store;
+        const KxxRest *rest = enqueue_assembly(g, jitter, &rest_store);
         {
             PhaseScope ps(c, PH_KSTAR, c->sweep_stream);
             launch_kstar(c->sweep_stream, g->X, k->P, 0, k->m_pad, g->h, Vws, ldv, g->n_pad);
@@ -1951,14 +2022,17 @@
         {
             PhaseScope ps(c, PH_CHOL);
             launch_cholesky(c->stream, c->side_stream, c->chol_events, g->A, g->lda, g->n_pad, g->invDt, g->info,
-                            chol_options(c, separate), &pipe, true);
-        }
-        HIP_TRY(hipEventRecord(c->ev_join, c->sweep_stream));
-        HIP_TRY(hipStreamWaitEvent(c->stream, c->ev_join, 0));
-        HIP_TRY(hipEventRecord(c->ev_join2, c->bulk_stream));
-        HIP_TRY(hipStreamWaitEvent(c->stream, c->ev_join2, 0));
+                            chol_options(c, separate), &pipe, true, rest);
+        }
+        if (!fin.fused) {
+            HIP_TRY(hipEventRecord(c->ev_join, c->sweep_stream));
+            HIP_TRY(hipStreamWaitEvent(c->stream, c->ev_join, 0));
+            HIP_TRY(hipEventRecord(c->ev_join2, c->bulk_stream));
+            HIP_TRY(hipStreamWaitEvent(c->stream, c->ev_join2, 0));
+        }
         HIP_TRY(hipGetLastError());
-        if (speculate) {
+        if (fin.fused) {
+        } else if (speculate) {
             rc = enqueue_finish(g, k, y_best, task, ei_jitter, cost, acq_out, mean_out, var_out, qbuf, mubuf, true, false);
             if (rc != CBO_OK) return rc;
         } else {
diff --git a/cbo_with_oop_amd/csrc/cbo_internal.h b/cbo_with_oop_amd/csrc/cbo_internal.h
--- a/cbo_with_oop_amd/csrc/cbo_internal.h
+++ b/cbo_with_oop_amd/csrc/cbo_internal.h
@@ -75,6 +75,14 @@
 void launch_zero_pair(hipStream_t s, double *a, double *b, int64_t n);
 void launch_rhs(hipStream_t s, const double *y, const double *pm, int64_t n, double *A, int64_t lda, int64_t n_pad,
                 int *zero = nullptr, int zero_count = 0);
+void launch_fit_head(hipStream_t s, const PointSet &X, const KernelHyper &h, double diag_add, double jitter, double *A,
+                     int64_t lda, int64_t n_pad, const double *y, int *zero, int zero_count);
+struct KxxRest {
+    const PointSet *X;
+    KernelHyper h;
+    double diag_add, jitter;
+};
+void launch_kxx_rest(hipStream_t s, const KxxRest &r, double *A, int64_t lda, int64_t n_pad, hipEvent_t done);
 void launch_kstar(hipStream_t s, const PointSet &X, const PointSet &C, int64_t c_begin, int64_t m_pad,
                   const KernelHyper &h, double *V, int64_t ldv, int64_t n_pad);
 
@@ -124,6 +132,7 @@
                             int64_t n32, int64_t m_pad, double *q);
 int run_mfma_f32_selftest(hipStream_t s, double *max_err);
 
+struct SweepFinish;
 struct SweepPipe {
     hipStream_t stream;
     hipStream_t bulk;
@@ -138,6 +147,7 @@
     std::vector<hipEvent_t> *events;
     void (*mark)(void *user, hipStream_t st, int begin, double flops);
     void *user;
+    const SweepFinish *finish = nullptr;
 };
 constexpr int kCholFlagSlots = 1024;
 constexpr int kCholFusedTimeout = -2147483647 - 1;
@@ -150,7 +160,7 @@
 };
 void launch_cholesky(hipStream_t s, hipStream_t side, std::vector<hipEvent_t> &events, double *A, int64_t lda,
                      int64_t n_pad, double *invDt, int *info_dev, const CholOptions &opt, const SweepPipe *pipe = nullptr,
-                     bool info_zeroed = false);
+                     bool info_zeroed = false, const KxxRest *kxx_rest = nullptr);
 inline int cholesky_info_ints(int64_t n_pad)
 {
     const int np = (int)(n_pad / 128);
@@ -184,7 +194,9 @@
 
 void launch_trsm_strips(hipStream_t s, const double *U, int64_t ldu, const double *invDt, double *V, int64_t ldv,
                         int64_t n, int64_t m_pad, const double *z, double *q, double *mu, bool accumulate = false,
-                        bool half_lds = false);
+                        bool half_lds = false, const SweepFinish *fin = nullptr);
+constexpr int kFinishMaxStrips = 2048;
+bool sweep_finish_fusable(int64_t n, int64_t m_pad);
 void launch_gemm_update(hipStream_t s, const double *U, int64_t ldu, const double *V, int64_t ldv, double *C,
                         int64_t ldc, int k0, int klen, int i0_begin, int i0_end, int64_t m_pad, bool upper_only,
                         const int *skip_if = nullptr);
@@ -275,6 +287,16 @@
     int task, include_noise, want_ei;
     const double *y_best_dev = nullptr;
 };
+struct SweepFinish {
+    AcqParams p;
+    const double *pm, *pv;
+    int64_t m, index_offset;
+    double *part_val; int64_t *part_idx;
+    int *ticket;
+    int strips;
+    double *best_val; int64_t *best_idx;
+    const int *status_src; int *status_dst;
+};
 void launch_acq(hipStream_t s, const double *q, const double *mu, const double *pm, const double *pv, int64_t m,
                 const AcqParams &p, double *mean_out, double *var_out, double *acq_out, double *part_val,
                 int64_t *part_idx, int64_t index_offset, int n_blocks);
diff --git a/cbo_with_oop_amd/csrc/kernels_chol.hip b/cbo_with_oop_amd/csrc/kernels_chol.hip
--- a/cbo_with_oop_amd/csrc/kernels_chol.hip
+++ b/cbo_with_oop_amd/csrc/kernels_chol.hip
@@ -935,7 +935,7 @@
     if (pipe.mark) pipe.mark(pipe.user, chain, 1, rows * rows * (double)pipe.m_pad);
     launch_trsm_strips(chain, A + (int64_t)t0 * lda + t0, lda, invDt + (int64_t)(t0 / 16) * 256,
                        pipe.V + (int64_t)t0 * pipe.ldv, pipe.ldv, (int64_t)n_pad - t0, pipe.m_pad, pipe.zvec + t0, pipe.q,
-                       pipe.mu, true, false);
+                       pipe.mu, true, false, pipe.finish);
     if (pipe.mark) pipe.mark(pipe.user, chain, 0, 0.0);
 }
 
@@ -946,7 +946,7 @@
 
 void launch_cholesky(hipStream_t s, hipStream_t side, std::vector<hipEvent_t> &events, double *A, int64_t lda,
                      int64_t n_pad, double *invDt, int *info_dev, const CholOptions &opt, const SweepPipe *pipe,
-                     bool info_zeroed)
+                     bool info_zeroed, const KxxRest *kxx_rest)
 {
     hipFuncSetAttribute(reinterpret_cast<const void *>(potrf_diag128_v2_kernel), hipFuncAttributeMaxDynamicSharedMemorySize,
                         (int)sizeof(Diag2Shared));
@@ -965,9 +965,11 @@
     if (!info_zeroed) hipLaunchKernelGGL(zero_ints_kernel, dim3(1), dim3(256), 0, s, info_dev, fused ? 1 + 2 * np : 1);
     int *flags = info_dev + 1;
     const int rcol = (int)n_pad;
-    event_slot(events, (size_t)(2 * np + 1));
+    event_slot(events, (size_t)(2 * np + 2));
     hipEventRecord(events[2 * np], s);
     hipStreamWaitEvent(side, events[2 * np], 0);
+    const hipEvent_t ev_kxx_rest = (kxx_rest && np > 1) ? events[2 * np + 2] : nullptr;
+    if (ev_kxx_rest) launch_kxx_rest(side, *kxx_rest, A, lda, n_pad, ev_kxx_rest);
     double *zvec = pipe ? pipe->zvec : nullptr;
     const bool lean_panel = !pipe;
     int pair = 0;
@@ -1009,6 +1011,7 @@
         };
         factor_panel(r0, n2, nullptr);
         if (n2 <= 0) { sweep_rows(r0, 128); break; }
+        if (k == 0 && ev_kxx_rest) hipStreamWaitEvent(s, ev_kxx_rest, 0);
         launch_syrk_rows(s, A, lda, r0, 128, n2, rcol, info_dev);
         const int r1 = r0 + 128;
         const int n3 = (int)n_pad - r1 - 128;
diff --git a/cbo_with_oop_amd/csrc/kernels_kmat.hip b/cbo_with_oop_amd/csrc/kernels_kmat.hip
--- a/cbo_with_oop_amd/csrc/kernels_kmat.hip
+++ b/cbo_with_oop_amd/csrc/kernels_kmat.hip
@@ -1,3 +1,5 @@
+#include <hip/hip_ext.h>
+
 #include "cbo_device.h"
 
 #pragma clang fp contract(off)
@@ -119,19 +121,20 @@
     double variance, lengthscale, diag_add, jitter;
     int symmetric, zero_diag;
     int sym_tiles;
+    int tile_begin;
     float *out32;
     const double *alpha;
     double *mu_part;
     int64_t ld_part;
 };
 
-template <int D, bool OUT32 = false>
-__global__ __launch_bounds__(256) void kmat_tile_kernel(KmatArgs a)
-{
-    int tj = blockIdx.x, ti = blockIdx.y;
+template <int D, bool OUT32>
+__device__ __forceinline__ void kmat_tile(const KmatArgs &a, int bx, int by)
+{
+    int tj = bx, ti = by;
     if (a.symmetric) {
         const int nt = a.sym_tiles;
-        const int t = blockIdx.x;
+        const int t = a.tile_begin + bx;
         ti = (int)((2.0 * nt + 1.0 - sqrt((2.0 * nt + 1.0) * (2.0 * nt + 1.0) - 8.0 * (double)t)) * 0.5);
         while (ti > 0 && ti * nt - ti * (ti - 1) / 2 > t) --ti;
         while ((ti + 1) * nt - (ti + 1) * ti / 2 <= t) ++ti;
@@ -234,29 +237,36 @@
     }
 }
 
+template <int D, bool OUT32 = false>
+__global__ __launch_bounds__(256) void kmat_tile_kernel(KmatArgs a)
+{
+    kmat_tile<D, OUT32>(a, (int)blockIdx.x, (int)blockIdx.y);
+}
+
 template <int D>
-static void launch_kmat_d(hipStream_t s, const KmatArgs &a, dim3 grid)
+static void launch_kmat_d(hipStream_t s, const KmatArgs &a, dim3 grid, hipEvent_t done)
 {
     if (a.out32) hipLaunchKernelGGL((kmat_tile_kernel<D, true>), grid, dim3(256), 0, s, a);
+    else if (done) hipExtLaunchKernelGGL((kmat_tile_kernel<D, false>), grid, dim3(256), 0, s, nullptr, done, 0, a);
     else hipLaunchKernelGGL((kmat_tile_kernel<D, false>), grid, dim3(256), 0, s, a);
 }
 
-static void launch_kmat(hipStream_t s, int d, const KmatArgs &a, dim3 grid)
+static void launch_kmat(hipStream_t s, int d, const KmatArgs &a, dim3 grid, hipEvent_t done = nullptr)
 {
     switch (d) {
-        case 1: launch_kmat_d<1>(s, a, grid); break;
-        case 2: launch_kmat_d<2>(s, a, grid); break;
-        case 3: launch_kmat_d<3>(s, a, grid); break;
-        case 4: launch_kmat_d<4>(s, a, grid); break;
-        case 5: launch_kmat_d<5>(s, a, grid); break;
-        case 6: launch_kmat_d<6>(s, a, grid); break;
-        case 7: launch_kmat_d<7>(s, a, grid); break;
-        default: launch_kmat_d<8>(s, a, grid); break;
-    }
-}
-
-void launch_kxx(hipStream_t s, const PointSet &X, const KernelHyper &h, double diag_add, double jitter, double *A,
-                int64_t lda, int64_t n_pad)
+        case 1: launch_kmat_d<1>(s, a, grid, done); break;
+        case 2: launch_kmat_d<2>(s, a, grid, done); break;
+        case 3: launch_kmat_d<3>(s, a, grid, done); break;
+        case 4: launch_kmat_d<4>(s, a, grid, done); break;
+        case 5: launch_kmat_d<5>(s, a, grid, done); break;
+        case 6: launch_kmat_d<6>(s, a, grid, done); break;
+        case 7: launch_kmat_d<7>(s, a, grid, done); break;
+        default: launch_kmat_d<8>(s, a, grid, done); break;
+    }
+}
+
+static KmatArgs kxx_args(const PointSet &X, const KernelHyper &h, double diag_add, double jitter, double *A, int64_t lda,
+                         int64_t n_pad)
 {
     KmatArgs a;
     a.rx = X.xs; a.ldr = X.ld; a.rsq = X.sq; a.rsv = X.sv;
@@ -265,8 +275,16 @@
     a.out = A; a.ldo = lda;
     a.variance = h.variance; a.lengthscale = h.lengthscale; a.diag_add = diag_add; a.jitter = jitter;
     a.symmetric = 1; a.zero_diag = h.zero_diag; a.out32 = nullptr; a.alpha = nullptr; a.mu_part = nullptr; a.ld_part = 0;
-    const int nt = (int)(n_pad / 64);
-    a.sym_tiles = nt;
+    a.sym_tiles = (int)(n_pad / 64);
+    a.tile_begin = 0;
+    return a;
+}
+
+void launch_kxx(hipStream_t s, const PointSet &X, const KernelHyper &h, double diag_add, double jitter, double *A,
+                int64_t lda, int64_t n_pad)
+{
+    const KmatArgs a = kxx_args(X, h, diag_add, jitter, A, lda, n_pad);
+    const int nt = a.sym_tiles;
     launch_kmat(s, X.d, a, dim3((unsigned)(nt * (nt + 1) / 2), 1));
 }
 
@@ -279,7 +297,7 @@
     a.n_rows = X.n; a.n_cols = C.ld; a.col_begin = c_begin;
     a.out = V; a.ldo = ldv;
     a.variance = h.variance; a.lengthscale = h.lengthscale; a.diag_add = 0.0; a.jitter = 0.0;
-    a.symmetric = 0; a.zero_diag = 0; a.sym_tiles = 0; a.out32 = nullptr; a.alpha = nullptr; a.mu_part = nullptr; a.ld_part = 0;
+    a.symmetric = 0; a.zero_diag = 0; a.sym_tiles = 0; a.tile_begin = 0; a.out32 = nullptr; a.alpha = nullptr; a.mu_part = nullptr; a.ld_part = 0;
     launch_kmat(s, X.d, a, dim3((unsigned)(m_pad / 64), (unsigned)(n_pad / 64)));
 }
 
@@ -304,10 +322,18 @@
     a.out = nullptr; a.ldo = ldv; a.out32 = V;
     a.alpha = alpha; a.mu_part = mu_part; a.ld_part = m_pad;
     a.variance = h.variance; a.lengthscale = h.lengthscale; a.diag_add = 0.0; a.jitter = 0.0;
-    a.symmetric = 0; a.zero_diag = 0; a.sym_tiles = 0;
+    a.symmetric = 0; a.zero_diag = 0; a.sym_tiles = 0; a.tile_begin = 0;
     launch_kmat(s, X.d, a, dim3((unsigned)(m_pad / 64), (unsigned)(n32 / 64)));
     hipLaunchKernelGGL(colsum_parts_kernel, dim3((unsigned)((m_pad + 255) / 256)), dim3(256), 0, s, mu_part, m_pad,
                        (int)(n32 / 64), m_pad, mu);
+}
+
+__device__ __forceinline__ double rhs_value(const double *__restrict__ y, const double *__restrict__ pm, int64_t n,
+                                            int64_t i, int c)
+{
+    double v = 0.0;
+    if (c == 0 && i < n) v = pm ? __dadd_rn(y[i], -pm[i]) : y[i];
+    return v;
 }
 
 __global__ __launch_bounds__(256) void rhs_kernel(const double *__restrict__ y, const double *__restrict__ pm,
@@ -320,9 +346,7 @@
     if (idx >= n_pad * kRhsCols) return;
     const int64_t i = idx / kRhsCols;
     const int c = (int)(idx % kRhsCols);
-    double v = 0.0;
-    if (c == 0 && i < n) v = pm ? __dadd_rn(y[i], -pm[i]) : y[i];
-    A[i * lda + n_pad + c] = v;
+    A[i * lda + n_pad + c] = rhs_value(y, pm, n, i, c);
 }
 
 void launch_rhs(hipStream_t s, const double *y, const double *pm, int64_t n, double *A, int64_t lda, int64_t n_pad,
@@ -331,6 +355,62 @@
     const int64_t total = n_pad * kRhsCols;
     hipLaunchKernelGGL(rhs_kernel, dim3((unsigned)((total + 255) / 256)), dim3(256), 0, s, y, pm, n, A, lda, n_pad, zero,
                        zero ? zero_count : 0);
+}
+
+template <int D>
+__global__ __launch_bounds__(256) void fit_head_kernel(KmatArgs a, int head_tiles, const double *__restrict__ y,
+                                                       const double *__restrict__ pm, int64_t n_pad,
+                                                       int *__restrict__ zero, int zero_count)
+{
+    const int b = (int)blockIdx.x;
+    if (b < head_tiles) {
+        kmat_tile<D, false>(a, b, 0);
+        return;
+    }
+    const int rb = b - head_tiles;
+    if (rb == 0)
+        for (int i = threadIdx.x; i < zero_count; i += 256) zero[i] = 0;
+    static_assert(kRhsCols == 64, "a workgroup of the strip is 64 rows of 64 columns");
+    const int c = threadIdx.x & 63;
+#pragma unroll 4
+    for (int r = threadIdx.x >> 6; r < 64; r += 4) {
+        const int64_t i = (int64_t)rb * 64 + r;
+        if (i < n_pad) a.out[i * a.ldo + n_pad + c] = rhs_value(y, pm, a.n_rows, i, c);
+    }
+}
+
+int kxx_head_tiles(int64_t n_pad) { return 2 * (int)(n_pad / 64) - 1; }
+
+void launch_fit_head(hipStream_t s, const PointSet &X, const KernelHyper &h, double diag_add, double jitter, double *A,
+                     int64_t lda, int64_t n_pad, const double *y, int *zero, int zero_count)
+{
+    const KmatArgs a = kxx_args(X, h, diag_add, jitter, A, lda, n_pad);
+    const int head = kxx_head_tiles(n_pad);
+    const dim3 grid((unsigned)(head + a.sym_tiles));
+    if (!zero) zero_count = 0;
+#define CBO_LAUNCH_HEAD(D) \
+    hipLaunchKernelGGL(fit_head_kernel<D>, grid, dim3(256), 0, s, a, head, y, X.pm, n_pad, zero, zero_count)
+    switch (X.d) {
+        case 1: CBO_LAUNCH_HEAD(1); break;
+        case 2: CBO_LAUNCH_HEAD(2); break;
+        case 3: CBO_LAUNCH_HEAD(3); break;
+        case 4: CBO_LAUNCH_HEAD(4); break;
+        case 5: CBO_LAUNCH_HEAD(5); break;
+        case 6: CBO_LAUNCH_HEAD(6); break;
+        case 7: CBO_LAUNCH_HEAD(7); break;
+        default: CBO_LAUNCH_HEAD(8); break;
+    }
+#undef CBO_LAUNCH_HEAD
+}
+
+void launch_kxx_rest(hipStream_t s, const KxxRest &r, double *A, int64_t lda, int64_t n_pad, hipEvent_t done)
+{
+    KmatArgs a = kxx_args(*r.X, r.h, r.diag_add, r.jitter, A, lda, n_pad);
+    const int nt = a.sym_tiles;
+    a.tile_begin = kxx_head_tiles(n_pad);
+    const int rest = nt * (nt + 1) / 2 - a.tile_begin;
+    if (rest <= 0) { if (done) hipEventRecord(done, s); return; }
+    launch_kmat(s, r.X->d, a, dim3((unsigned)rest, 1), done);
 }
 
 __global__ __launch_bounds__(256) void zero_pair_kernel(double *__restrict__ a, double *__restrict__ b, int64_t n)
diff --git a/cbo_with_oop_amd/csrc/kernels_trsm.hip b/cbo_with_oop_amd/csrc/kernels_trsm.hip
--- a/cbo_with_oop_amd/csrc/kernels_trsm.hip
+++ b/cbo_with_oop_amd/csrc/kernels_trsm.hip
@@ -1,7 +1,7 @@
 #include <cstdlib>
 #include <type_traits>
 
-#include "cbo_internal.h"
+#include "cbo_device.h"
 
 namespace cbo {
 
@@ -719,13 +719,61 @@
     unsigned b_dst;
 };
 
-template <bool SWEEP>
+__device__ __forceinline__ void pair_finish(const SweepFinish &f, bool holder, int64_t col, double q, double mu)
+{
+#pragma clang fp contract(off)
+    __shared__ double red_v[8];
+    __shared__ int64_t red_i[8];
+    __shared__ int last_flag;
+    double bv = -INFINITY;
+    int64_t bi = kNoIndex;
+    if (holder && col < f.m) {
+        const bool causal = f.pm != nullptr;
+        double mean, var;
+        posterior_of(q, mu, causal ? f.pm[col] : 0.0, causal ? f.pv[col] : 0.0, causal, f.p, mean, var);
+        bv = acquisition_of(mean, var, f.p);
+        bi = col + f.index_offset;
+    }
+    wave_argmax(bv, bi);
+    const int tid = threadIdx.x;
+    if ((tid & 63) == 0) { red_v[tid >> 6] = bv; red_i[tid >> 6] = bi; }
+    __syncthreads();
+    if (tid == 0) {
+        for (int w = 1; w < 8; ++w)
+            if (better(red_v[w], red_i[w], bv, bi)) { bv = red_v[w]; bi = red_i[w]; }
+        f.part_val[blockIdx.x] = bv;
+        f.part_idx[blockIdx.x] = bi;
+        __threadfence();
+        last_flag = (atomicAdd(f.ticket, 1) == f.strips - 1) ? 1 : 0;
+    }
+    __syncthreads();
+    if (last_flag == 0 || tid >= 64) return;
+    __threadfence();
+    const int status = (tid == 0 && f.status_src) ? __builtin_nontemporal_load(f.status_src) : 0;
+    bv = -INFINITY;
+    bi = kNoIndex;
+    for (int b = tid; b < f.strips; b += 64) {
+        const double v = __builtin_nontemporal_load(&f.part_val[b]);
+        const int64_t i = __builtin_nontemporal_load(&f.part_idx[b]);
+        if (better(v, i, bv, bi)) { bv = v; bi = i; }
+    }
+    wave_argmax(bv, bi);
+    if (tid == 0) {
+        *f.best_val = bv;
+        *f.best_idx = bi;
+        if (f.status_src) *f.status_dst = status;
+        *f.ticket = 0;
+    }
+}
+
+template <bool SWEEP, bool FIN = false>
 __global__ __launch_bounds__(512) void trsm_pair_kernel(const double *__restrict__ U, int64_t ldu,
                                                         const double *__restrict__ invDt, double *V, int64_t ldv,
                                                         int n, const double *__restrict__ z,
                                                         double *__restrict__ q_out, double *__restrict__ mu_out,
-                                                        int accumulate)
+                                                        int accumulate, const SweepFinish *__restrict__ fin)
 {
+    static_assert(SWEEP || !FIN, "only a sweep has q and mu to finish from");
     __shared__ __align__(16) double lds[kNBuf * (kPA + kPBd)];
     __shared__ __align__(16) double zl[SWEEP ? 2 * kPB : 2];
     __shared__ __align__(16) double handbuf[SWEEP ? 4 * 64 * 2 : 2];
@@ -796,6 +844,7 @@
         for (int i = 0; i < kPDma; ++i) issue_one(c, buf, i);
     };
 
+    double qfin = 0.0, mfin = 0.0;
     auto run = [&](auto role_tag) __attribute__((always_inline)) {
         constexpr int H = decltype(role_tag)::value;
         d4 acc[kT];
@@ -1159,9 +1208,14 @@
             q_out[colw + lc] = qtot;
             mu_out[colw + lc] = mtot;
         }
+        if constexpr (FIN && H == 1) {
+            qfin = qtot;
+            mfin = mtot;
+        }
     };
     if (h == 0) run(std::integral_constant<int, 0>{});
     else run(std::integral_constant<int, 1>{});
+    if constexpr (FIN) pair_finish(*fin, h == 1 && kq == 0, colw + lc, qfin, mfin);
 }
 
 constexpr int kAccMoves = kT * 4;
@@ -1309,11 +1363,30 @@
     __builtin_amdgcn_s_barrier();
 }
 
+static bool pair_form(int64_t n)
+{
+    static const bool pairs = [] {
+        const char *e = getenv("CBO_HIP_STRIP_FORM");
+        return !(e && atoi(e) == 8);
+    }();
+    return pairs && n >= kPB && n % kPB == 0;
+}
+
+bool sweep_finish_fusable(int64_t n, int64_t m_pad)
+{
+    return n > 0 && pair_form(n) && m_pad > 0 && m_pad / kStrip <= kFinishMaxStrips;
+}
+
 void launch_trsm_strips(hipStream_t s, const double *U, int64_t ldu, const double *invDt, double *V, int64_t ldv,
                         int64_t n, int64_t m_pad, const double *z, double *q, double *mu, bool accumulate,
-                        bool half_lds)
+                        bool half_lds, const SweepFinish *fin)
 {
     if (n <= 0 || m_pad <= 0) return;
+    if (fin) {
+        hipLaunchKernelGGL((trsm_pair_kernel<true, true>), dim3((unsigned)(m_pad / kStrip)), dim3(512), 0, s, U, ldu, invDt, V,
+                           ldv, (int)n, z, q, mu, accumulate ? 1 : 0, fin);
+        return;
+    }
     const dim3 grid((unsigned)(m_pad / kStrip));
     const int acc = accumulate ? 1 : 0;
     if (half_lds) {
@@ -1323,15 +1396,11 @@
             hipLaunchKernelGGL((trsm_strip_kernel<false, 16>), grid, dim3(256), 0, s, U, ldu, invDt, V, ldv, (int)n, z, q, mu, 0);
         return;
     }
-    static const bool pairs = [] {
-        const char *e = getenv("CBO_HIP_STRIP_FORM");
-        return !(e && atoi(e) == 8);
-    }();
-    if (pairs && n >= kPB && n % kPB == 0) {
+    if (pair_form(n)) {
         if (q != nullptr)
-            hipLaunchKernelGGL((trsm_pair_kernel<true>), grid, dim3(512), 0, s, U, ldu, invDt, V, ldv, (int)n, z, q, mu, acc);
+            hipLaunchKernelGGL((trsm_pair_kernel<true>), grid, dim3(512), 0, s, U, ldu, invDt, V, ldv, (int)n, z, q, mu, acc, nullptr);
         else
-            hipLaunchKernelGGL((trsm_pair_kernel<false>), grid, dim3(512), 0, s, U, ldu, invDt, V, ldv, (int)n, z, q, mu, 0);
+            hipLaunchKernelGGL((trsm_pair_kernel<false>), grid, dim3(512), 0, s, U, ldu, invDt, V, ldv, (int)n, z, q, mu, 0, nullptr);
         return;
     }
     if (q != nullptr)
```

After: 3.072 million, median of 2. Within noise of the previous version (+0.2%).
